# LSimon95/megatts2

Measured on AMD Instinct MI355X. Metric: mel-frames/sec (whole node), higher is better.
Workload: dtype f32; 1 GPU; C3: B=32/GPU x 1 GPU, Np=70, Tp=431, Tm=431; stages vqpe+mrte+adm+plm+decoder+vocoder; forced durations; weights=synthetic (name-seeded), parallelism=dp1 (utterance shards, one RCCL all-gather of mels per step)

## Files before the change

include/megatts2_hip.h:

```cpp
#ifndef MEGATTS2_HIP_H
#define MEGATTS2_HIP_H

#include <stddef.h>
#include <stdint.h>

#ifdef __cplusplus
extern "C" {
#endif

typedef struct mt2_model mt2_model;

typedef struct mt2_config {
    int32_t mel_bins, mrte_hidden, mrte_kernel, mrte_stride, mrte_n_layer, mrte_n_stack, mrte_n_block;
    int32_t content_ff_dim, content_n_heads, content_n_layers, phone_vocab;
    int32_t vq_mel_bins, vq_stride, vq_hidden, vq_kernel, vq_n_layers, vq_n_stacks, vq_n_blocks, vq_bins, vq_dim;
    int32_t dec_kernel, dec_hidden, dec_n_stack, dec_n_block;
    int32_t plm_layers, plm_heads, plm_vq_dim, plm_tc_dim, plm_bins;
    int32_t adm_layers, adm_heads, adm_emb_dim, adm_tc_dim, adm_tc_emb_dim;
    int32_t hg_in_dim, hg_init_channels, hg_n_up, hg_up_rates[8], hg_up_kernels[8];
    int32_t hg_n_res, hg_res_kernels[4], hg_res_dilations[4][3];
    float hg_slope;
    int32_t max_positions;
    int32_t hg_inference_padding;
    int32_t hg_reflect_pad;
// ... 158 lines not shown

#define MT2_LIMITER_FIELDS 24
#define MT2_LIMITER_TILE 1024
#define MT2_LIMITER_MAX_HALF_WINDOW 1024
#define MT2_LIMITER_MAX_PASSES 4
int mt2_limiter_query(int sample_rate, long long L, double window_ms, int* half_window, int* tile, long long* workspace_bytes);
int mt2_limiter_window(int sample_rate, double window_ms, float* w );
int mt2_limit_true_peak(mt2_model* m, void* stream, const float* wav , const int32_t* lens , int L_max, int B,
                        int sample_rate, double pre_gain_db, double ceiling_dbtp, double window_ms, float* out ,
                        float* gain , float* need , double* stats );
int mt2_loudness_normalize_limited(mt2_model* m, void* stream, const float* wav , const int32_t* lens , int L_max,
                                   int B, int sample_rate, double target_lufs, double ceiling_dbtp, double window_ms, int passes,
                                   float* out , float* gain , float* need ,
                                   double* stats );

#define MT2_RUN_PLM 1
#define MT2_RUN_VOCODER 2
#define MT2_SKIP_ADM 4
#define MT2_PROMPT_VQPE 8
int mt2_synthesize_batch(mt2_model* m, void* stream, const int64_t* phone, const int32_t* phone_lens ,
                         int Np_max, const float* prompt_mel, const int32_t* prompt_lens , int Tp_max,
                         int B, const int32_t* forced_dur , const int64_t* forced_codes, int Tq_cap,
                         int flags, float* mel, int Tm_cap, int32_t* mel_lens , int32_t* dur_out,
                         int64_t* codes_out, float* wav, int64_t* prompt_codes);

int mt2_synthesize_prompt_conditioned(mt2_model* m, void* stream, const int64_t* phone, const int32_t* phone_lens ,
                                      int Np_max, const float* prompt_mel, const int32_t* prompt_lens , int Tp_max, int B,
                                      const int64_t* prompt_phone, const int32_t* prompt_phone_lens , int Npp_max,
                                      const int32_t* prompt_dur , const int32_t* forced_dur , int Tq_cap, int flags,
                                      float* mel, int Tm_cap, int32_t* mel_lens , int32_t* dur_out, int64_t* codes_out,
                                      float* wav, int64_t* prompt_codes);
int mt2_synthesize_batch_sampled(mt2_model* m, void* stream, const int64_t* phone, const int32_t* phone_lens ,
                                 int Np_max, const float* prompt_mel, const int32_t* prompt_lens , int Tp_max,
                                 int B, const int32_t* forced_dur , const int64_t* forced_codes, int Tq_cap,
                                 int flags, float* mel, int Tm_cap, int32_t* mel_lens , int32_t* dur_out,
                                 int64_t* codes_out, float* wav, int64_t* prompt_codes, const mt2_sampling* sampling);
int mt2_synthesize_prompt_conditioned_sampled(mt2_model* m, void* stream, const int64_t* phone,
                                              const int32_t* phone_lens , int Np_max, const float* prompt_mel,
                                              const int32_t* prompt_lens , int Tp_max, int B,
                                              const int64_t* prompt_phone, const int32_t* prompt_phone_lens ,
                                              int Npp_max, const int32_t* prompt_dur ,
                                              const int32_t* forced_dur , int Tq_cap, int flags, float* mel,
                                              int Tm_cap, int32_t* mel_lens , int32_t* dur_out, int64_t* codes_out,
                                              float* wav, int64_t* prompt_codes, const mt2_sampling* sampling);

int mt2_set_option(mt2_model* m, const char* name, int value);
int mt2_get_option(mt2_model* m, const char* name, int* value);
int mt2_set_ar_groups(mt2_model* m, int groups);

int mt2_set_profiling(mt2_model* m, int enable);
int mt2_last_stage_ms(mt2_model* m, const char** names, float* ms, int cap);

int mt2_op_gemm(void* stream, const float* X, int ldx, int Rx, const int32_t* rowbase, int a_mul, int shift0,
                int taps, int dil, int Cin, const float* W, int ldw, const float* bias, const float* R, int ldr,
                const int32_t* valid, float* C, int ldc, int M, int N, int pro_act, float pro_slope, int epi_act,
                float out_scale, int force_cfg);
int mt2_op_gemm_x6(void* stream, const float* X, int ldx, int Rx, int shift0, int taps, int dil, int Cin, const float* W,
                   const void* W3, const float* bias, const float* R, int ldr, const int32_t* valid, float* C, int ldc,
                   int M, int N, int pro_act, float pro_slope, int epi_act, int force_cfg);
int mt2_op_gemm_x3h(void* stream, const float* X, int ldx, int Rx, int shift0, int taps, int dil, int Cin, const float* W,
                    const void* W3, const void* Wh, const float* wh_inv, const float* bias, const float* R, int ldr,
                    const int32_t* valid, float* C, int ldc, int M, int N, int pro_act, float pro_slope, int epi_act, int force_cfg,
                    int32_t* range_flag);
int mt2_x3h_split(const float* W, long long rows, long long row_len, uint16_t* planes, float* inv);
int mt2_x3h_group_planes(long long row_len, long long w_off, long long ldw, long long strideW, long long groups, int32_t* form,
                         long long* wh_off, long long* wh_ldb, long long* wh_gstride, long long* inv_off, long long* wh_inv_stride);
typedef struct mt2_gemm_desc {
    int32_t struct_bytes;
    const float* X; long long strideX; int32_t ldx, Rx;
    const int32_t* rowbase; int32_t a_mul, shift0, taps, dil, Cin;
    const float* W; long long strideW; int32_t ldw;
    const void* W3; long long w3_plane;
    const void* Wh; const float* wh_inv; long long wh_ldb, wh_gstride, wh_inv_stride;
    int32_t a_planes;
    const float* bias; long long strideB;
    const float* R; long long strideR; int32_t ldr;
    const int32_t* valid;
    float* C; long long strideC; int32_t ldc;
    int32_t M, N, groups;
    int32_t pro_act; float pro_slope; int32_t epi_act; float out_scale;
    int32_t force_cfg;
    int32_t* range_flag;
    int32_t* cfg_out;
} mt2_gemm_desc;
int mt2_op_gemm_grouped(void* stream, const mt2_gemm_desc* d);
int mt2_x3h_guard(mt2_model* m, int* tripped);
int mt2_op_gemm_x6_ln(void* stream, const float* X, int ldx, int Rx, int a_mul, int shift0, const float* W, const void* W3,
                      const float* bias, const float* R, int ldr, float* C, int ldc, int M, int N, int K, int epi_act,
                      int force_cfg, float* stat_out, int32_t* stat_nt, int32_t* stat_w, const float* ln_stat, int ln_nt,
                      int ln_w, const float* ln_s, float ln_eps);
int mt2_op_tile_major(void* stream, const float* W, int N, int K, float* out);
int mt2_op_gemm_tm(void* stream, const float* X, long long x_gstride, int ldx, int Rx, int a_mul, int shift0, const float* Wtm,
                   int Kw, int n0, int k0, long long w_gstride, int groups, const float* bias, const float* R, int ldr,
                   const int32_t* valid, float* C, long long c_gstride, int ldc, int M, int N, int K, int pro_act, float pro_slope,
                   int epi_act, const float* ln_gamma, const float* ln_beta, float ln_eps);
int mt2_op_gemm_tm_pairs(void* stream, const float* X, int ldx, int Rx, int a_mul, int shift0, const float* Wtm, int Kw,
                         const float* bias, const float* R, int ldr, float* C, int ldc, int M, int N, int K, int epi_act,
                         const float* ln_gamma, const float* ln_beta, float ln_eps, float* stat_out, const float* ln_stat, int ln_nt);
int mt2_op_layernorm(void* stream, const float* x, int ldx, const float* gamma, const float* beta, const float* R1,
                     int ldr1, const int32_t* valid, float* out, int ldo, int M, int C, float eps, int act);
int mt2_op_layernorm_ex(void* stream, const float* x, int ldx, const float* gamma, const float* beta, int rows_per_group,
                        const float* R1, int ldr1, int r1_rows, const float* R2, int ldr2, const int32_t* valid, int valid_rows,
                        float* out, int ldo, int M, int C, float eps, int act, int out_planes, int32_t* x3h_flag);
int mt2_op_ln_reduce(void* stream, const float* parts, long long pstride, int S, const float* bias, const float* R, int ldr,
                     const float* gamma, const float* beta, float* xout, int ldx, float* hout, int ldh, int M, int C, float eps,
                     int h_planes, int32_t* x3h_flag);
int mt2_op_row(void* stream, const char* op, void* const* ptrs, int nptrs, const long long* ints, int nints, const float* flts,
               int nflts);
int mt2_op_sample_rows(void* stream, const float* logits, int ld, int N, int A, const mt2_sampling* s, const uint64_t* seeds_dev,
                       const int32_t* positions_dev, int64_t* out);
int mt2_op_sample_mix_rows(void* stream, const float* logits, int ld, int N, int A, const mt2_sampling* s,
                           const uint64_t* seeds_dev, const int32_t* positions_dev, const float* gamma_dev, int64_t* out);
int mt2_op_attention(void* stream, const float* Q, int ldq, const float* K, int ldk, const float* V, int ldv,
                     float* O, int ldo, const int32_t* q_start, const int32_t* q_len, const int32_t* kv_start,
                     const int32_t* kv_len, int B, int H, int D, int max_qlen, float scale);
int mt2_op_attention_tuned(void* stream, const float* Q, int ldq, const float* K, int ldk, const float* V, int ldv,
                           float* O, int ldo, const int32_t* q_start, const int32_t* q_len, const int32_t* kv_start,
                           const int32_t* kv_len, int B, int H, int D, int max_qlen, float scale, int lds_min_qlen,
                           int lds_waves, int x6_min_qlen, int max_kvlen);
int mt2_op_attention_x3h(void* stream, const float* Q, int ldq, const float* K, int ldk, const float* V, int ldv,
                         float* O, int ldo, const int32_t* q_start, const int32_t* q_len, const int32_t* kv_start,
                         const int32_t* kv_len, int B, int H, int D, int max_qlen, float scale, int lds_waves, int max_kvlen,
                         int32_t* range_flag);
enum { MT2_ATTN_NONE = 0, MT2_ATTN_GENERIC = 1, MT2_ATTN_REG = 2, MT2_ATTN_DS = 3, MT2_ATTN_LDS = 4, MT2_ATTN_X6 = 5, MT2_ATTN_X3H = 6 };
typedef struct mt2_attn_desc {
    int32_t struct_bytes;
    const float* Q; int32_t ldq;
    const float* K; int32_t ldk;
    const float* V; int32_t ldv;
    float* O; int32_t ldo;
    const int32_t* q_start; const int32_t* q_len; const int32_t* kv_start; const int32_t* kv_len; const int32_t* o_start;
    int32_t u_qstride, u_qlen, u_kvstride, u_kvlen, u_ostride;
    int32_t B, H, D, max_qlen, max_kvlen; float scale;
    int32_t lds_min_qlen, x6_min_qlen, lds_waves, ds_short, x3h, o_planes;
    int32_t* range_flag;
    int32_t* kernel_out;
} mt2_attn_desc;
int mt2_op_attention_desc(void* stream, const mt2_attn_desc* d);
int mt2_attention_route(const mt2_attn_desc* d, int32_t* err, int32_t* kernel, int32_t* tmpl, int32_t* launch, long long* lds);
int mt2_gemm_trace_begin(mt2_model* m);
int mt2_gemm_trace_end(mt2_model* m, int cap, const char** names, int64_t* launches, double* flops, double* ms);
int mt2_gemm_trace_shapes(mt2_model* m, char* buf, int cap, int top);
int mt2_form_log_begin(mt2_model* m);
int mt2_form_log_end(mt2_model* m, char* buf, int cap);
int mt2_gemm_config_count(void);
const char* mt2_gemm_config_name(int idx);
int mt2_gemm_route(int M, int N, int K, int taps, int dil, int groups, int pro_act, int operands, int misaligned, int force_cfg,
                   int x3h, int* err, int* cfg, int* variant, long long* lds, int* planes);
int mt2_conv_pair_route(int R, int C, int taps, int dil, int flags, int pair_fuse, int x3h, int* err, long long* lds, int* grid,
                        int* block, int* bm, int* bmo);
int mt2_op_conv_pair(void* stream, const float* X, int ldx, int R, int C, int taps, int dil, float slope, const void* Wh1,
                     const float* inv1, const float* bias1, const void* Wh2, const float* inv2, const float* bias2,
                     const int32_t* valid, float* Y, int ldy, int pair_fuse, int32_t* range_flag);
int mt2_up_mrf_route(int R, int ch, int stride, int flags, int up_fuse, int x3h, int off, int* err, long long* lds, int* grid, int* block,
                     int* bm);
int mt2_op_up_mrf(void* stream, const float* X0, const float* X1, const float* X2, int ldx, int R, int ch, float scale, float slope,
                  const void* Wh, const float* inv, const float* bias, const int32_t* valid, float* Y, int ldy, int up_fuse,
                  int32_t* range_flag);
int mt2_op_gemm_x3h_ln(void* stream, const float* X, int ldx, int Rx, int a_mul, int shift0, const float* W, const void* W3,
                       const void* Wh, const float* wh_inv, const float* bias, const float* R, int ldr, float* C, int ldc, int M, int N,
                       int K, int epi_act, int force_cfg, float* stat_out, int32_t* stat_nt, int32_t* stat_w, const float* ln_stat,
                       int ln_nt, int ln_w, const float* ln_s, float ln_eps);
int mt2_bench_gemm(void* stream, int M, int N, int K, int taps, int dil, int flags, int force_cfg, int iters,
                   int w_copies, float* avg_ms, char* cfg_name, int cfg_name_cap, double* sustained_ghz);

#ifdef __cplusplus
}
#endif
#endif
```

megatts2_amd/csrc/capi.inc:

```

#include <climits>

namespace mt2 {
extern thread_local std::string g_last_error;
void finalize_model(mt2_model& m);
}

using namespace mt2;

#define MT2_API_BEGIN try {
#define MT2_API_END                                 \
    ::CallScope::verdict_of_open_call();            \
    return 0;                                       \
    }                                               \
    catch (const std::exception& e) {               \
        g_last_error = e.what();                    \
        return -1;                                  \
    }                                               \
    catch (...) {                                   \
        g_last_error = "unknown error";             \
        return -1;                                  \
    }

enum Need { NEED_G = 1, NEED_ADM = 2, NEED_PLM = 4, NEED_VOC = 8 };
// ... 232 lines not shown
    need((m.hg_post.k - 1) / 2);
    return (int)gap;
}

int mt2_workspace_query(const mt2_model* m, int B, int Np_max, int Tp_max, int Tm_cap, int flags, size_t* bytes) {
    MT2_API_BEGIN
    MT2_REQUIRE(m != nullptr && bytes != nullptr && B >= 1 && Np_max >= 1 && Tp_max >= 1 && Tm_cap >= 1, "bad arguments");
    const mt2_config& cfg = m->cfg;
    auto rows = [&](long long len, int gap) { return (long long)gap + (long long)B * (len + gap); };
    auto enc = [&](long long M, long long d, long long ff) {
        return M * (5 * d + ff + 128) + std::max(256ll * 32 * 64 + 16ll * 32 * d, 8 * M * d) + 7 * 64;
    };
    auto ar = [&](long long d, long long ff, long long L, int stage_groups) {
        const long long M = (long long)B * L;
        const int G = std::max(1, std::min(stage_groups > 0 ? stage_groups : m->ar_groups, B));
        return M * d + 3 * M * d + (long long)B * d + G * enc(0, d, ff) + enc(M + 2ll * B * G, d, ff) - enc(0, d, ff);
    };
    const long long H = cfg.mrte_hidden, st = cfg.mrte_stride;
    const long long FR = rows(Tp_max, prompt_mel_gap(cfg)), XR = rows((Tp_max - 1) / st + 1, mel_context_gap(cfg)), PR = rows(Np_max, phone_gap(cfg));
    long long f = 0;
    f += 16 * (FR + XR + PR) + 64;
    f += FR * cfg.mel_bins + FR * H + 4 * FR * H * cfg.mrte_n_layer + XR * H * cfg.mrte_n_layer;
    f += 4 * XR * H * cfg.mrte_n_layer + 2 * XR * H;
    f += PR * H + enc(PR, H, cfg.content_ff_dim) + 2 * XR * H + 2 * PR * H;
    if (!(flags & MT2_SKIP_ADM)) {
        f += PR * cfg.adm_tc_emb_dim + (long long)B * (Np_max + 1) + 8ll * B;
        f += ar(cfg.adm_emb_dim + cfg.adm_tc_emb_dim, 4ll * cfg.adm_emb_dim, Np_max, m->adm_groups);
    }
    const long long DR = rows(Tm_cap, decoder_gap(cfg)), DIN = H + cfg.vq_dim, Tq = (Tm_cap + cfg.vq_stride - 1) / cfg.vq_stride;
    f += 8 * DR + 4ll * B * Tq + DR * DIN + (long long)B * Tq * H + (long long)B * Np_max;
    if (flags & MT2_RUN_PLM) {
        const long long d = cfg.plm_vq_dim + cfg.plm_tc_dim;
        f += 2ll * B * (Tq + 1) + 2ll * B * Tq + 8ll * B + (long long)B * cfg.plm_bins + 2ll * B;
        f += ar(d, 4 * d, Tq, m->plm_groups);
    }
    f += DR * cfg.dec_hidden * 5 + DR * cfg.mel_bins;
    if (flags & MT2_PROMPT_VQPE) {
        const long long VR = rows(Tp_max, vqpe_gap(cfg)), QR = rows((Tp_max + cfg.vq_stride - 1) / cfg.vq_stride, vqpe_gap(cfg));
        const long long C = cfg.vq_hidden, G = cfg.vq_n_layers;
        f += 16 * (VR + QR) + VR * cfg.mel_bins + VR * C + 4 * VR * C * G + G * QR * C + 4 * QR * C * G + QR * C;
        f += QR * cfg.vq_dim + QR * cfg.vq_bins + 2 * QR;
    }
    if (flags & MT2_RUN_VOCODER) {
        const long long pad = cfg.hg_inference_padding;
        long long R = rows(Tm_cap + 2 * pad, vocoder_gap(*m)), ch = cfg.hg_init_channels;
        f += 4 * R + R * cfg.mel_bins + R * ch;
        for (int i = 0; i < cfg.hg_n_up; ++i) {
            R *= cfg.hg_up_rates[i];
            ch /= 2;
            f += R + 14 * R * ch;
        }
        f += R + 4ll * B + 64;
    }
    *bytes = (size_t)f * sizeof(float) + (size_t)400 * 256 + ((size_t)8 << 20);
    MT2_API_END
}

static int* option_slot(mt2_model* m, const std::string& n) {
    if (n == "ar_groups") return &m->ar_groups;
    if (n == "adm_groups") return &m->adm_groups;
    if (n == "plm_groups") return &m->plm_groups;
    if (n == "force_gemm_config") return &m->opts.force_cfg;
    if (n == "t_ks4") return &m->opts.t_ks4;
    if (n == "t_ks2") return &m->opts.t_ks2;
    if (n == "t32") return &m->opts.t32;
    if (n == "t32x32") return &m->opts.t32x32;
    if (n == "t_x6_256") return &m->opts.t_x6_256;
    if (n == "t_x6_128") return &m->opts.t_x6_128;
    if (n == "t_x3h_128") return &m->opts.t_x3h_128;
    if (n == "x3h") return &m->opts.x3h;
    if (n == "x6_ks") return &m->opts.x6_ks;
    if (n == "voc_streams") return &m->opts.voc_streams;
    if (n == "ldr_prio") return &m->opts.ldr_prio;
    if (n == "skinny_rows") return &m->opts.skinny_rows;
    if (n == "skinny_nw") return &m->opts.skinny_nw;
    if (n == "skinny_pairs") return &m->opts.skinny_pairs;
    if (n == "attn_lds_min") return &m->opts.attn_lds_min;
    if (n == "attn_x6_min") return &m->opts.attn_x6_min;
    if (n == "ln_pairs_adm") return &m->opts.ln_pairs_adm;
    if (n == "ln_pairs_maxm") return &m->opts.ln_pairs_maxm;
    if (n == "a_planes") return &m->opts.a_planes;
    if (n == "pair_fuse") return &m->opts.pair_fuse;
    if (n == "up_fuse") return &m->opts.up_fuse;
    return nullptr;
}
static bool* option_flag(mt2_model* m, const std::string& n) {
    if (n == "splitk") return &m->opts.splitk;
    if (n == "stage_markers") return &m->opts.markers;
    if (n == "win_conv") return &m->opts.win_conv;
    if (n == "x6_conv") return &m->opts.x6_conv;
    if (n == "x6_gemm") return &m->opts.x6_gemm;
    if (n == "skinny_tm") return &m->opts.skinny_tm;
    if (n == "ldr64") return &m->opts.ldr64;
    return nullptr;
}
int mt2_set_option(mt2_model* m, const char* name, int value) {
    MT2_API_BEGIN
    MT2_REQUIRE(m != nullptr && name != nullptr, "null argument");
    std::lock_guard<std::mutex> lk(m->call_mutex);
    const std::string n(name);
    if (n == "ar_groups") MT2_REQUIRE(value >= 1 && value <= 8, "ar_groups must be in 1..8");
    if (int* p = option_slot(m, n)) *p = value;
    else if (bool* q = option_flag(m, n)) *q = value != 0;
    else throw Error("unknown option " + n);
    MT2_API_END
}
int mt2_get_option(mt2_model* m, const char* name, int* value) {
    MT2_API_BEGIN
    MT2_REQUIRE(m != nullptr && name != nullptr && value != nullptr, "null argument");
    const std::string n(name);
    if (int* p = option_slot(m, n)) *value = *p;
    else if (bool* q = option_flag(m, n)) *value = *q ? 1 : 0;
    else throw Error("unknown option " + n);
    MT2_API_END
}
int mt2_set_ar_groups(mt2_model* m, int groups) { return mt2_set_option(m, "ar_groups", groups); }
int mt2_set_profiling(mt2_model* m, int enable) {
    MT2_API_BEGIN
    MT2_REQUIRE(m != nullptr, "null model handle");
    m->profiling = enable != 0;
    MT2_API_END
}
int mt2_last_stage_ms(mt2_model* m, const char** names, float* ms, int cap) {
    if (!m) return -1;
    const int n = (int)m->stage_ms.size();
    for (int i = 0; i < n && i < cap; ++i) {
        names[i] = m->stage_names[i].c_str();
        ms[i] = m->stage_ms[i];
    }
    return n;
}

int mt2_mrte_tc_latent(mt2_model* m, void* stream, const int64_t* phone, const int32_t* phone_lens, int Np_max,
                       const float* mel, const int32_t* mel_lens, int Tp_max, int B, float* out) {
    MT2_API_BEGIN
    require_ready(m, NEED_G);
    MT2_REQUIRE(B >= 1, "empty batch");
    MT2_CALL(m, stream);
    const int H = m->cfg.mrte_hidden;
    TcResult r = tc_latent_rows(c, phone, phone_lens, Np_max, mel, mel_lens, Tp_max, B);
    IntPlan ip;
    const int o_map = plan_rowmap(ip, r.P, Np_max);
    ip.upload(c.ws, c.m.pinned(), c.s);
    MT2_HIP(hipMemsetAsync(out, 0, sizeof(float) * (size_t)B * Np_max * H, c.s));
    MT2_HIP(launch_unpack_rows(r.rows, H, H, Np_max, 0, ip.dev(o_map), out, r.P.R, c.s));
    ids_verdict(c);
    MT2_API_END
}

int mt2_mrte_mel_context(mt2_model* m, void* stream, const float* mel, const int32_t* mel_lens, int Tp_max, int B,
                         float* out, int Tc_max) {
    MT2_API_BEGIN
    require_ready(m, NEED_G);
    MT2_REQUIRE(B >= 1, "empty batch");
    MT2_CALL(m, stream);
    const mt2_config& cfg = m->cfg;
    IntPlan ip;
    MelPlan mp = plan_mel(ip, cfg, mel_lens, B, Tp_max, Tc_max);
    MT2_REQUIRE(mp.X.maxlen <= Tc_max, "Tc_max too small");
    ip.upload(c.ws, c.m.pinned(), c.s);
    bind_rows(ip, mp.oF, mp.F);
    bind_rows(ip, mp.oX, mp.X);
    float* xmel = c.ws.get<float>((size_t)mp.F.R * cfg.mel_bins);
    MT2_HIP(launch_pack_rows(mel, cfg.mel_bins, Tp_max, 0, ip.dev(mp.o_rowmapF), xmel, cfg.mel_bins, mp.F.R, c.s));
    float* ctx = mel_context_rows(c, xmel, cfg.mel_bins, mp.F, mp.X, ip.dev(mp.o_rowbase));
    const int H = cfg.mrte_hidden;
// ... 826 lines not shown
    float* xdec = rows + (size_t)pp.D.R * DIN;
    MT2_HIP(launch_gather_rows(tc.rows, H, ip.dev(pp.o_tcmap), rows, DIN, H, pp.D.R, c.s));
    MT2_HIP(launch_gather_rows(tc.rows, H, ip.dev(fp.o_tcmap), xdec, DIN, H, fp.D.R, c.s));
    float* cond = c.ws.get<float>((size_t)qr * H);
    MT2_HIP(launch_pool_max(rows, DIN, ip.dev(o_first), ip.dev(o_cnt), cond, H, H, qr, c.s));
    st.mark("regulate");
    join_vqpe_side(c);
    int64_t* cdev = codes_buffer(c, codes_out, B, Tq_cap);
    ArPrefix pre;
    pre.P = P; pre.data = prompt_codes; pre.stride = (Tp_max + pool - 1) / pool;
    plm_run(c, cond, H, q0, total.data(), B, cdev, Tq_cap, nullptr, 0, pre, sampling);
    st.mark("plm");
    decode_and_vocode(c, st, xdec, fp, ip, cdev, flags, mel, Tm_cap, wav, B);
    st.finish();
    MT2_API_END
}
int mt2_synthesize_prompt_conditioned(mt2_model* m, void* stream, const int64_t* phone, const int32_t* phone_lens, int Np_max,
                                      const float* prompt_mel, const int32_t* prompt_lens, int Tp_max, int B,
                                      const int64_t* prompt_phone, const int32_t* prompt_phone_lens, int Npp_max,
                                      const int32_t* prompt_dur, const int32_t* forced_dur, int Tq_cap, int flags, float* mel,
                                      int Tm_cap, int32_t* mel_lens, int32_t* dur_out, int64_t* codes_out, float* wav,
                                      int64_t* prompt_codes) {
    return mt2_synthesize_prompt_conditioned_sampled(m, stream, phone, phone_lens, Np_max, prompt_mel, prompt_lens, Tp_max, B,
                                                     prompt_phone, prompt_phone_lens, Npp_max, prompt_dur, forced_dur, Tq_cap,
                                                     flags, mel, Tm_cap, mel_lens, dur_out, codes_out, wav, prompt_codes,
                                                     nullptr);
}


int mt2_gemm_trace_begin(mt2_model* m) {
    MT2_API_BEGIN
    MT2_REQUIRE(m != nullptr, "null model handle");
    std::lock_guard<std::mutex> lk(m->call_mutex);
    for (auto& r : m->opts.trace) { (void)hipEventDestroy(r.e0); (void)hipEventDestroy(r.e1); }
    m->opts.trace.clear();
    m->opts.trace_on = true;
    MT2_API_END
}
int mt2_gemm_trace_end(mt2_model* m, int cap, const char** names, int64_t* launches, double* flops, double* ms) {
    if (!m) return -1;
    std::lock_guard<std::mutex> lk(m->call_mutex);
    return gemm_trace_collect(m->opts, cap, names, launches, flops, ms);
}
int mt2_gemm_trace_shapes(mt2_model* m, char* buf, int cap, int top) {
    if (!m || !buf || cap <= 0) return -1;
    std::lock_guard<std::mutex> lk(m->call_mutex);
    return gemm_trace_shapes(m->opts, buf, cap, top);
}
int mt2_form_log_begin(mt2_model* m) {
    MT2_API_BEGIN
    MT2_REQUIRE(m != nullptr, "null model handle");
    std::lock_guard<std::mutex> lk(m->call_mutex);
    m->form_log.clear();
    m->form_kind = nullptr;
    m->form_log_on = true;
    MT2_API_END
}
int mt2_form_log_end(mt2_model* m, char* buf, int cap) {
    if (!m || !buf || cap <= 0) return -1;
    std::lock_guard<std::mutex> lk(m->call_mutex);
    m->form_log_on = false;
    m->form_kind = nullptr;
    size_t need = 0;
    for (const std::string& l : m->form_log) need += l.size() + 1;
    int off = -1;
    if (need < (size_t)cap) {
        off = 0;
        for (const std::string& l : m->form_log) {
            std::memcpy(buf + off, l.data(), l.size());
            off += (int)l.size();
            buf[off++] = '\n';
        }
        buf[off] = 0;
    }
    m->form_log.clear();
    m->form_log.shrink_to_fit();
    return off;
}
int mt2_gemm_config_count(void) { return gemm_num_configs(); }
const char* mt2_gemm_config_name(int idx) { return gemm_config_name(idx); }

int mt2_gemm_route(int M, int N, int K, int taps, int dil, int groups, int pro_act, int operands, int misaligned, int force_cfg,
                   int x3h, int* err, int* cfg, int* variant, long long* lds, int* planes) {
    alignas(128) static char dummy[12 * 128];
    const auto ptr = [&](int slot, int bit) { return (void*)(dummy + 128 * slot + ((misaligned & bit) ? 4 : 0)); };
    GemmP p{};
    const int Cin = taps > 0 ? K / taps : K;
    p.X = (const float*)ptr(0, 512); p.ldx = Cin; p.Rx = M + taps * dil; p.a_mul = 1; p.taps = taps; p.dil = dil; p.Cin = Cin;
    p.W = (const float*)ptr(1, 0); p.ldw = K; p.C = (float*)ptr(2, 1024); p.ldc = N; p.M = M; p.N = N; p.K = K; p.groups = groups;
    p.strideX = (long long)p.Rx * Cin; p.strideW = (long long)N * K; p.strideC = (long long)M * N; p.strideB = N; p.strideR = (long long)M * N;
    p.pro_act = pro_act; p.out_scale = 1.0f;
    if (operands & 1) p.W3 = ptr(3, 1);
    if (operands & 2) { p.Wh = ptr(4, 2); p.wh_inv = (const float*)ptr(5, 0); }
    if (operands & 4) { p.Wtm = (const float*)ptr(6, 4); p.tm_kb = K / 64; }
    if (operands & 8) p.stat_out = (float*)ptr(7, 8);
    if (operands & 16) { p.ln_stat = (const float*)ptr(8, 16); p.ln_g = p.ln_b = (const float*)ptr(9, 0); p.ln_w = 64; p.ln_nt = K / 64; }
    if (operands & 32) { p.R = (const float*)ptr(10, 32); p.ldr = N; }
    if (operands & 64) p.rowbase = (const int*)ptr(11, 64);
    p.a_planes = (operands & 128) ? 1 : 0;
    p.c_planes = (operands & 256) ? 1 : 0;
    EngineOpts o;
    o.force_cfg = force_cfg;
    o.x3h = x3h;
    const GemmRoute r = gemm_route(p, o);
    if (err) *err = (int)r.err;
    if (cfg) *cfg = r.cfg;
    if (variant) *variant = r.variant;
    if (lds) *lds = (long long)r.lds;
    if (planes) *planes = (gemm_takes_planes(p, o) ? 1 : 0) | (gemm_writes_planes(p, o) ? 2 : 0);
    return 0;
}

int mt2_conv_pair_route(int R, int C, int taps, int dil, int flags, int pair_fuse, int x3h, int* err, long long* lds, int* grid,
                        int* block, int* bm, int* bmo) {
    alignas(128) static char dummy[8 * 128];
    PairP p{};
    p.X = (const float*)dummy; p.ldx = C; p.R = R; p.C = C; p.taps = taps; p.dil = dil; p.slope = 0.1f;
    if (!(flags & 2)) { p.Wh1 = dummy + 128; p.inv1 = (const float*)(dummy + 256); p.Wh2 = dummy + 384; p.inv2 = (const float*)(dummy + 512); }
    p.bias1 = (const float*)(dummy + 640); p.bias2 = (const float*)(dummy + 768);
    p.wh_ldb = 4ll * (((long long)taps * C + 31) / 32 * 32);
    p.Y = (float*)(dummy + 896 + ((flags & 8) ? 4 : 0)); p.ldy = C;
    p.reflect = (flags & 1) ? 1 : 0;
    if ((flags & 4) && R > 0) p.ldx = (int)((((1ll << 31) / 4 + R - 1) / R + 3) & ~3ll);
    EngineOpts o;
    o.pair_fuse = pair_fuse;
    o.x3h = x3h;
    const PairRoute r = conv_pair_route(p, o);
    if (err) *err = (int)r.err;
    if (lds) *lds = (long long)r.lds;
    if (grid) *grid = (int)r.grid;
    if (block) *block = (int)r.block;
    if (bm) *bm = r.bm;
    if (bmo) *bmo = r.bmo;
    return 0;
}
int mt2_op_conv_pair(void* stream, const float* X, int ldx, int R, int C, int taps, int dil, float slope, const void* Wh1,
                     const float* inv1, const float* bias1, const void* Wh2, const float* inv2, const float* bias2,
                     const int32_t* valid, float* Y, int ldy, int pair_fuse, int32_t* range_flag) {
    MT2_API_BEGIN
    PairP p{};
    p.X = X; p.ldx = ldx; p.R = R; p.C = C; p.taps = taps; p.dil = dil; p.slope = slope;
    p.Wh1 = Wh1; p.inv1 = inv1; p.bias1 = bias1; p.Wh2 = Wh2; p.inv2 = inv2; p.bias2 = bias2;
    p.wh_ldb = 4ll * (((long long)taps * C + 31) / 32 * 32);
    p.valid = valid; p.Y = Y; p.ldy = ldy;
    EngineOpts o;
    o.pair_fuse = pair_fuse;
    o.x3h_flag = range_flag;
    MT2_HIP(launch_conv_pair(p, (hipStream_t)stream, &o));
    MT2_API_END
}

int mt2_up_mrf_route(int R, int ch, int stride, int flags, int up_fuse, int x3h, int off, int* err, long long* lds, int* grid, int* block,
                     int* bm) {
    alignas(128) static char dummy[8 * 128];
    UpMrfP p{};
    p.X0 = (const float*)dummy; p.X1 = (flags & 32) ? nullptr : (const float*)(dummy + 128); p.X2 = (const float*)(dummy + 256);
    p.ldx = ch; p.R = R; p.ch = ch; p.stride = stride; p.scale = 1.0f / 3.0f; p.slope = 0.1f;
    if (!(flags & 1)) { p.Wh = dummy + 384 + ((flags & 8) ? 16 : 0); p.inv = (const float*)(dummy + 512); }
    p.bias = (const float*)(dummy + 640 + ((flags & 128) ? 4 : 0));
    p.wh_ldb = 8ll * ch;
    p.Y = (float*)(dummy + 768 + ((flags & 4) ? 4 : 0)); p.ldy = ch;
    if ((flags & 2) && R > 0) p.ldx = (int)((((1ll << 31) / 4 + R - 1) / R + 3) & ~3ll);
    if (flags & 16) p.ldx = ch + 2;
    if (flags & 64) p.ldy = ch - 4;
    EngineOpts o;
    o.up_fuse = up_fuse;
    o.x3h = x3h;
    if (off & 1) o.win_conv = false;
    if (off & 2) o.x6_conv = false;
    if (off & 4) o.force_cfg = 0;
    if (off & 8) o.ldr64 = true;
    const UpMrfRoute r = up_mrf_route(p, o);
    if (err) *err = (int)r.err;
    if (lds) *lds = (long long)r.lds;
    if (grid) *grid = (int)r.grid;
    if (block) *block = (int)r.block;
    if (bm) *bm = r.bm;
    return 0;
}
int mt2_op_up_mrf(void* stream, const float* X0, const float* X1, const float* X2, int ldx, int R, int ch, float scale, float slope,
                  const void* Wh, const float* inv, const float* bias, const int32_t* valid, float* Y, int ldy, int up_fuse,
                  int32_t* range_flag) {
    MT2_API_BEGIN
    UpMrfP p{};
    p.X0 = X0; p.X1 = X1; p.X2 = X2; p.ldx = ldx; p.R = R; p.ch = ch; p.stride = 2; p.scale = scale; p.slope = slope;
    p.Wh = Wh; p.inv = inv; p.bias = bias; p.wh_ldb = 8ll * ch;
    p.valid = valid; p.Y = Y; p.ldy = ldy;
    EngineOpts o;
    o.up_fuse = up_fuse;
    o.x3h_flag = range_flag;
    MT2_HIP(launch_up_mrf(p, (hipStream_t)stream, &o));
    MT2_API_END
}

int mt2_op_gemm(void* stream, const float* X, int ldx, int Rx, const int32_t* rowbase, int a_mul, int shift0,
                int taps, int dil, int Cin, const float* W, int ldw, const float* bias, const float* R, int ldr,
                const int32_t* valid, float* C, int ldc, int M, int N, int pro_act, float pro_slope, int epi_act,
                float out_scale, int force_cfg) {
    MT2_API_BEGIN
    GemmP p{};
    p.X = X; p.ldx = ldx; p.Rx = Rx; p.rowbase = rowbase; p.a_mul = a_mul ? a_mul : 1; p.shift0 = shift0;
    p.taps = taps; p.dil = dil; p.Cin = Cin; p.W = W; p.ldw = ldw; p.bias = bias; p.R = R; p.ldr = ldr;
    p.valid = valid; p.C = C; p.ldc = ldc; p.M = M; p.N = N; p.K = taps * Cin; p.groups = 1;
    p.pro_act = pro_act; p.pro_slope = pro_slope; p.epi_act = epi_act; p.out_scale = out_scale;
    EngineOpts o;
    o.force_cfg = force_cfg;
    MT2_HIP(launch_gemm(p, (hipStream_t)stream, &o));
    MT2_API_END
}

int mt2_op_gemm_x6(void* stream, const float* X, int ldx, int Rx, int shift0, int taps, int dil, int Cin, const float* W,
                   const void* W3, const float* bias, const float* R, int ldr, const int32_t* valid, float* C, int ldc,
                   int M, int N, int pro_act, float pro_slope, int epi_act, int force_cfg) {
    MT2_API_BEGIN
    GemmP p{};
    p.X = X; p.ldx = ldx; p.Rx = Rx; p.a_mul = 1; p.shift0 = shift0; p.taps = taps; p.dil = dil; p.Cin = Cin; p.W = W;
    p.W3 = W3; p.ldw = taps * Cin; p.bias = bias; p.R = R; p.ldr = ldr; p.valid = valid; p.C = C; p.ldc = ldc; p.M = M;
    p.N = N; p.K = taps * Cin; p.groups = 1; p.pro_act = pro_act; p.pro_slope = pro_slope; p.epi_act = epi_act;
    p.out_scale = 1.0f;
    EngineOpts o;
    o.force_cfg = force_cfg;
    MT2_HIP(launch_gemm(p, (hipStream_t)stream, &o));
    MT2_API_END
}

int mt2_op_gemm_x3h(void* stream, const float* X, int ldx, int Rx, int shift0, int taps, int dil, int Cin, const float* W,
                    const void* W3, const void* Wh, const float* wh_inv, const float* bias, const float* R, int ldr,
                    const int32_t* valid, float* C, int ldc, int M, int N, int pro_act, float pro_slope, int epi_act, int force_cfg,
                    int32_t* range_flag) {
    MT2_API_BEGIN
    GemmP p{};
    p.X = X; p.ldx = ldx; p.Rx = Rx; p.a_mul = 1; p.shift0 = shift0; p.taps = taps; p.dil = dil; p.Cin = Cin; p.W = W;
    p.W3 = W3; p.Wh = Wh; p.wh_inv = wh_inv; p.ldw = taps * Cin; p.bias = bias; p.R = R; p.ldr = ldr; p.valid = valid; p.C = C;
    p.ldc = ldc; p.M = M; p.N = N; p.K = taps * Cin; p.groups = 1; p.pro_act = pro_act; p.pro_slope = pro_slope; p.epi_act = epi_act;
    p.out_scale = 1.0f;
    EngineOpts o;
    if (force_cfg >= 4000) { p.c_planes = 1; force_cfg -= 4000; }
    if (force_cfg >= 2000) { p.a_planes = 1; force_cfg -= 2000; }
    o.ldr64 = force_cfg >= 1000;
    o.force_cfg = force_cfg >= 1000 ? force_cfg - 1000 : force_cfg;
    o.x3h_flag = range_flag;
    MT2_HIP(launch_gemm(p, (hipStream_t)stream, &o));
    MT2_API_END
}
int mt2_x3h_split(const float* W, long long rows, long long row_len, uint16_t* planes, float* inv) {
    MT2_API_BEGIN
    MT2_REQUIRE(W && planes && inv && rows > 0 && row_len > 0, "bad arguments");
    x3h_split_rows(W, (size_t)rows, (size_t)row_len, planes, inv);
    MT2_API_END
}
int mt2_x3h_group_planes(long long row_len, long long w_off, long long ldw, long long strideW, long long groups, int32_t* form,
                         long long* wh_off, long long* wh_ldb, long long* wh_gstride, long long* inv_off, long long* wh_inv_stride) {
    MT2_API_BEGIN
    MT2_REQUIRE(row_len > 0 && w_off >= 0 && groups >= 1 && form && wh_off && wh_ldb && wh_gstride && inv_off && wh_inv_stride,
                "bad arguments");
    const X3hGroupPlanes g = x3h_group_planes(row_len, w_off, ldw, strideW, groups);
    *form = g.form; *wh_off = g.wh_off; *wh_ldb = g.wh_ldb; *wh_gstride = g.wh_gstride; *inv_off = g.inv_off;
    *wh_inv_stride = g.wh_inv_stride;
    MT2_API_END
}

int mt2_op_gemm_grouped(void* stream, const mt2_gemm_desc* d) {
    MT2_API_BEGIN
    MT2_REQUIRE(d != nullptr, "null descriptor");
    MT2_REQUIRE(d->struct_bytes == (int32_t)sizeof(mt2_gemm_desc), "descriptor size mismatch");
    if (d->cfg_out) *d->cfg_out = -1;
    GemmP p{};
    p.X = d->X; p.strideX = d->strideX; p.ldx = d->ldx; p.Rx = d->Rx;
    p.rowbase = d->rowbase; p.a_mul = d->a_mul; p.shift0 = d->shift0; p.taps = d->taps; p.dil = d->dil; p.Cin = d->Cin;
    p.W = d->W; p.strideW = d->strideW; p.ldw = d->ldw;
    p.W3 = d->W3; p.w3_plane = d->w3_plane;
    p.Wh = d->Wh; p.wh_inv = d->wh_inv; p.wh_ldb = d->wh_ldb; p.wh_gstride = d->wh_gstride; p.wh_inv_stride = d->wh_inv_stride;
    p.a_planes = d->a_planes;
    p.bias = d->bias; p.strideB = d->strideB; p.R = d->R; p.strideR = d->strideR; p.ldr = d->ldr; p.valid = d->valid;
    p.C = d->C; p.strideC = d->strideC; p.ldc = d->ldc;
    p.M = d->M; p.N = d->N; p.K = d->taps * d->Cin; p.groups = d->groups;
    p.pro_act = d->pro_act; p.pro_slope = d->pro_slope; p.epi_act = d->epi_act; p.out_scale = d->out_scale;
    MT2_REQUIRE(p.X && p.W && p.C && p.taps >= 1 && p.dil >= 1 && p.a_mul >= 1 && p.groups >= 1, "bad arguments");
    EngineOpts o;
    o.force_cfg = d->force_cfg;
    o.x3h_flag = d->range_flag;
    if (d->cfg_out) *d->cfg_out = gemm_route(p, o).cfg;
    MT2_HIP(launch_gemm(p, (hipStream_t)stream, &o));
    MT2_API_END
}

static int op_gemm_ln_impl(void* stream, const float* X, int ldx, int Rx, int a_mul, int shift0, const float* W, const void* W3,
                           const void* Wh, const float* wh_inv, const float* bias, const float* R, int ldr, float* C, int ldc, int M,
                           int N, int K, int epi_act, int force_cfg, float* stat_out, int32_t* stat_nt, int32_t* stat_w,
                           const float* ln_stat, int ln_nt, int ln_w, const float* ln_s, float ln_eps);
int mt2_op_gemm_x6_ln(void* stream, const float* X, int ldx, int Rx, int a_mul, int shift0, const float* W, const void* W3,
                      const float* bias, const float* R, int ldr, float* C, int ldc, int M, int N, int K, int epi_act,
                      int force_cfg, float* stat_out, int32_t* stat_nt, int32_t* stat_w, const float* ln_stat, int ln_nt,
                      int ln_w, const float* ln_s, float ln_eps) {
    return op_gemm_ln_impl(stream, X, ldx, Rx, a_mul, shift0, W, W3, nullptr, nullptr, bias, R, ldr, C, ldc, M, N, K, epi_act, force_cfg,
                           stat_out, stat_nt, stat_w, ln_stat, ln_nt, ln_w, ln_s, ln_eps);
}
int mt2_op_gemm_x3h_ln(void* stream, const float* X, int ldx, int Rx, int a_mul, int shift0, const float* W, const void* W3,
                       const void* Wh, const float* wh_inv, const float* bias, const float* R, int ldr, float* C, int ldc, int M, int N,
                       int K, int epi_act, int force_cfg, float* stat_out, int32_t* stat_nt, int32_t* stat_w, const float* ln_stat,
                       int ln_nt, int ln_w, const float* ln_s, float ln_eps) {
    return op_gemm_ln_impl(stream, X, ldx, Rx, a_mul, shift0, W, W3, Wh, wh_inv, bias, R, ldr, C, ldc, M, N, K, epi_act, force_cfg,
                           stat_out, stat_nt, stat_w, ln_stat, ln_nt, ln_w, ln_s, ln_eps);
}
static int op_gemm_ln_impl(void* stream, const float* X, int ldx, int Rx, int a_mul, int shift0, const float* W, const void* W3,
                           const void* Wh, const float* wh_inv, const float* bias, const float* R, int ldr, float* C, int ldc, int M,
                           int N, int K, int epi_act, int force_cfg, float* stat_out, int32_t* stat_nt, int32_t* stat_w,
                           const float* ln_stat, int ln_nt, int ln_w, const float* ln_s, float ln_eps) {
    MT2_API_BEGIN
    GemmP p{};
    p.Wh = Wh; p.wh_inv = wh_inv;
    p.X = X; p.ldx = ldx; p.Rx = Rx; p.a_mul = a_mul ? a_mul : 1; p.shift0 = shift0; p.taps = 1; p.dil = 1; p.Cin = K; p.W = W;
    p.W3 = W3; p.ldw = K; p.bias = bias; p.R = R; p.ldr = ldr; p.C = C; p.ldc = ldc; p.M = M; p.N = N; p.K = K; p.groups = 1;
    p.epi_act = epi_act; p.out_scale = 1.0f; p.stat_out = stat_out;
    if (ln_stat) { p.pro_act = 5; p.ln_stat = ln_stat; p.ln_nt = ln_nt; p.ln_w = ln_w; p.ln_g = ln_s; p.ln_eps = ln_eps; }
    EngineOpts o;
    o.ldr64 = force_cfg >= 1000;
    o.force_cfg = force_cfg >= 1000 ? force_cfg - 1000 : force_cfg;
    const hipError_t e = launch_gemm(p, (hipStream_t)stream, &o);
    MT2_REQUIRE(e != hipErrorNotSupported, "this tile configuration has no pair-fed LayerNorm form");
    MT2_HIP(e);
    if (stat_nt) *stat_nt = o.last_stat_nt;
    if (stat_w) *stat_w = o.last_stat_w;
    MT2_API_END
}

int mt2_op_tile_major(void* stream, const float* W, int N, int K, float* out) {
    MT2_API_BEGIN
    MT2_REQUIRE(W && out && N > 0 && K > 0 && N % 16 == 0 && K % 64 == 0, "tile-major layout needs N % 16 == 0 and K % 64 == 0");
    MT2_HIP(launch_tile_major(W, N, K, out, (hipStream_t)stream));
    MT2_API_END
}

int mt2_op_gemm_tm(void* stream, const float* X, long long x_gstride, int ldx, int Rx, int a_mul, int shift0, const float* Wtm,
                   int Kw, int n0, int k0, long long w_gstride, int groups, const float* bias, const float* R, int ldr,
                   const int32_t* valid, float* C, long long c_gstride, int ldc, int M, int N, int K, int pro_act, float pro_slope,
                   int epi_act, const float* ln_gamma, const float* ln_beta, float ln_eps) {
    MT2_API_BEGIN
    MT2_REQUIRE(X && Wtm && C && Kw % 64 == 0 && n0 % 16 == 0 && k0 % 64 == 0 && groups >= 1, "bad arguments");
    GemmP p{};
    p.X = X; p.strideX = x_gstride; p.ldx = ldx; p.Rx = Rx; p.a_mul = a_mul ? a_mul : 1; p.shift0 = shift0; p.taps = 1; p.dil = 1;
    p.Cin = K; p.K = K; p.W = nullptr; p.strideW = w_gstride; p.ldw = Kw; p.Wtm = Wtm; p.tm_n0 = n0 / 16; p.tm_k0 = k0 / 64;
    p.tm_kb = Kw / 64; p.bias = bias; p.R = R; p.ldr = ldr; p.valid = valid; p.C = C; p.strideC = c_gstride; p.ldc = ldc;
    p.M = M; p.N = N; p.groups = groups; p.pro_act = ln_gamma ? 3 : (pro_act & 0xff); p.pro_slope = pro_slope; p.epi_act = epi_act;
    p.sk_nw = (pro_act & 0x100) ? 8 : 16;
    p.out_scale = 1.0f; p.ln_g = ln_gamma; p.ln_b = ln_beta; p.ln_eps = ln_eps;
    MT2_REQUIRE(gemm_skinny_tm_eligible(p, 64), "shape not served by the tile-major weight-streaming kernel");
    MT2_HIP(launch_gemm_skinny_tm(p, (hipStream_t)stream));
    MT2_API_END
}

int mt2_op_gemm_tm_pairs(void* stream, const float* X, int ldx, int Rx, int a_mul, int shift0, const float* Wtm, int Kw,
                         const float* bias, const float* R, int ldr, float* C, int ldc, int M, int N, int K, int epi_act,
                         const float* ln_gamma, const float* ln_beta, float ln_eps, float* stat_out, const float* ln_stat, int ln_nt) {
    MT2_API_BEGIN
    MT2_REQUIRE(X && Wtm && C && Kw % 64 == 0, "bad arguments");
    GemmP p{};
    p.X = X; p.ldx = ldx; p.Rx = Rx; p.a_mul = a_mul ? a_mul : 1; p.shift0 = shift0; p.taps = 1; p.dil = 1; p.Cin = K; p.K = K;
    p.ldw = Kw; p.Wtm = Wtm; p.tm_kb = Kw / 64; p.bias = bias; p.R = R; p.ldr = ldr; p.C = C; p.ldc = ldc; p.M = M; p.N = N; p.groups = 1;
    p.pro_act = ln_gamma ? 3 : 0; p.epi_act = epi_act; p.out_scale = 1.0f; p.ln_g = ln_gamma; p.ln_b = ln_beta; p.ln_eps = ln_eps;
    p.stat_out = stat_out; p.ln_stat = ln_stat; p.ln_nt = ln_nt; p.ln_w = ln_stat ? 16 : 0;
    EngineOpts o;
    hipError_t e = launch_gemm(p, (hipStream_t)stream, &o);
    MT2_HIP(e);
    MT2_REQUIRE(!stat_out || o.last_stat_w == 16, "the launch did not take the tile-major route with the statistics epilogue");
    MT2_API_END
}

int mt2_op_layernorm(void* stream, const float* x, int ldx, const float* gamma, const float* beta, const float* R1,
                     int ldr1, const int32_t* valid, float* out, int ldo, int M, int C, float eps, int act) {
    MT2_API_BEGIN
    LnP p{};
    p.x = x; p.ldx = ldx; p.gamma = gamma; p.beta = beta; p.R1 = R1; p.ldr1 = ldr1; p.valid = valid;
    p.out = out; p.ldo = ldo; p.M = M; p.C = C; p.eps = eps; p.act = act >= 100 ? act - 100 : act;
    p.out_planes = act >= 100 ? 1 : 0;
    MT2_HIP(launch_layernorm(p, (hipStream_t)stream));
    MT2_API_END
}

int mt2_op_layernorm_ex(void* stream, const float* x, int ldx, const float* gamma, const float* beta, int rows_per_group,
                        const float* R1, int ldr1, int r1_rows, const float* R2, int ldr2, const int32_t* valid, int valid_rows,
                        float* out, int ldo, int M, int C, float eps, int act, int out_planes, int32_t* x3h_flag) {
    MT2_API_BEGIN
    LnP p{};
    p.x = x; p.ldx = ldx; p.gamma = gamma; p.beta = beta; p.rows_per_group = rows_per_group;
    p.R1 = R1; p.ldr1 = ldr1; p.r1_rows = r1_rows; p.R2 = R2; p.ldr2 = ldr2; p.valid = valid; p.valid_rows = valid_rows;
    p.out = out; p.ldo = ldo; p.M = M; p.C = C; p.eps = eps; p.act = act; p.out_planes = out_planes; p.x3h_flag = x3h_flag;
    MT2_HIP(launch_layernorm(p, (hipStream_t)stream));
    MT2_API_END
}

int mt2_op_ln_reduce(void* stream, const float* parts, long long pstride, int S, const float* bias, const float* R, int ldr,
                     const float* gamma, const float* beta, float* xout, int ldx, float* hout, int ldh, int M, int C, float eps,
                     int h_planes, int32_t* x3h_flag) {
    MT2_API_BEGIN
    LnReduceP p{};
    p.parts = parts; p.pstride = pstride; p.S = S; p.bias = bias; p.R = R; p.ldr = ldr; p.gamma = gamma; p.beta = beta;
    p.xout = xout; p.ldx = ldx; p.hout = hout; p.ldh = ldh; p.M = M; p.C = C; p.eps = eps; p.h_planes = h_planes;
    p.x3h_flag = x3h_flag;
// ... 192 lines not shown
int mt2_bench_gemm(void* stream, int M, int N, int K, int taps, int dil, int flags, int force_cfg, int iters,
                   int w_copies, float* avg_ms, char* cfg_name, int cfg_name_cap, double* sustained_ghz) {
    MT2_API_BEGIN
    MT2_REQUIRE(taps >= 1 && K % taps == 0 && (K / taps) % 4 == 0 && iters >= 1 && dil >= 1, "bad GEMM shape");
    if (w_copies < 1) w_copies = 1;
    hipStream_t s = (hipStream_t)stream;
    const int Cin = K / taps;
    float *X, *W, *C, *R = nullptr, *bias = nullptr;
    int* valid = nullptr;
    MT2_HIP(hipMalloc((void**)&X, sizeof(float) * ((size_t)M + taps * dil) * Cin));
    MT2_HIP(hipMalloc((void**)&W, sizeof(float) * (size_t)N * K * w_copies));
    MT2_HIP(hipMalloc((void**)&C, sizeof(float) * (size_t)M * N));
    std::vector<float> h(std::max(std::max(((size_t)M + taps * dil) * Cin, (size_t)N * K), (size_t)M * N));
    unsigned rng = 12345u;
    for (auto& v : h) { rng = rng * 1664525u + 1013904223u; v = ((rng >> 8) & 0xffff) / 32768.0f - 1.0f; }
    MT2_HIP(hipMemcpy(X, h.data(), sizeof(float) * ((size_t)M + taps * dil) * Cin, hipMemcpyHostToDevice));
    if (flags & 2) {
        MT2_HIP(hipMalloc((void**)&R, sizeof(float) * (size_t)M * N));
        MT2_HIP(hipMalloc((void**)&bias, sizeof(float) * (size_t)N));
        MT2_HIP(hipMalloc((void**)&valid, sizeof(int) * (size_t)M));
        MT2_HIP(hipMemcpy(R, h.data(), sizeof(float) * (size_t)M * N, hipMemcpyHostToDevice));
        MT2_HIP(hipMemcpy(bias, h.data(), sizeof(float) * (size_t)N, hipMemcpyHostToDevice));
        std::vector<int> ones(M, 1);
        MT2_HIP(hipMemcpy(valid, ones.data(), sizeof(int) * (size_t)M, hipMemcpyHostToDevice));
    }
    for (int i = 0; i < w_copies; ++i)
        MT2_HIP(hipMemcpy(W + (size_t)i * N * K, h.data(), sizeof(float) * (size_t)N * K, hipMemcpyHostToDevice));
    uint16_t* W3 = nullptr;
    const size_t wn = (size_t)N * K, wall = wn * w_copies;
    {
        std::vector<uint16_t> pl(3 * wall);
        for (size_t i = 0; i < wn; ++i) {
            float r = h[i];
            for (int k = 0; k < 3; ++k) {
                uint32_t bits;
                std::memcpy(&bits, &r, 4);
                bits &= 0xffff0000u;
                float top;
                std::memcpy(&top, &bits, 4);
                for (int cidx = 0; cidx < w_copies; ++cidx) pl[k * wall + cidx * wn + i] = (uint16_t)(bits >> 16);
                r -= top;
            }
        }
        MT2_HIP(hipMalloc((void**)&W3, pl.size() * sizeof(uint16_t)));
        MT2_HIP(hipMemcpy(W3, pl.data(), pl.size() * sizeof(uint16_t), hipMemcpyHostToDevice));
    }
    uint16_t* Wh = nullptr;
    float* wh_inv = nullptr;
    const size_t whn = (size_t)N * 2 * x3h_padded_k((size_t)K);
    {
        std::vector<uint16_t> one(whn), pl(whn * w_copies);
        std::vector<float> inv((size_t)N);
        x3h_split_rows(h.data(), (size_t)N, (size_t)K, one.data(), inv.data());
        for (int cidx = 0; cidx < w_copies; ++cidx) std::memcpy(pl.data() + cidx * whn, one.data(), whn * sizeof(uint16_t));
        MT2_HIP(hipMalloc((void**)&Wh, pl.size() * sizeof(uint16_t)));
        MT2_HIP(hipMemcpy(Wh, pl.data(), pl.size() * sizeof(uint16_t), hipMemcpyHostToDevice));
        MT2_HIP(hipMalloc((void**)&wh_inv, inv.size() * sizeof(float)));
        MT2_HIP(hipMemcpy(wh_inv, inv.data(), inv.size() * sizeof(float), hipMemcpyHostToDevice));
    }
    float* Wtm = nullptr;
    const bool tm = M <= 64 && taps == 1 && N % 16 == 0 && K % 64 == 0;
    if (tm) {
        MT2_HIP(hipMalloc((void**)&Wtm, sizeof(float) * wall));
        for (int i = 0; i < w_copies; ++i) MT2_HIP(launch_tile_major(W + (size_t)i * wn, N, K, Wtm + (size_t)i * wn, s));
    }
    GemmP p{};
    p.X = X; p.ldx = Cin; p.Rx = M + taps * dil; p.a_mul = 1; p.shift0 = 0; p.taps = taps; p.dil = dil; p.Cin = Cin;
    p.Wh = Wh; p.wh_inv = wh_inv;
    p.W = W; p.W3 = W3; p.w3_plane = (long long)wall; p.ldw = K; p.C = C; p.ldc = N; p.M = M; p.N = N; p.K = K; p.groups = 1;
    p.out_scale = 1.0f;
    if (tm) { p.Wtm = Wtm; p.tm_kb = K / 64; }
    if (flags & 1) { p.pro_act = ACT_LRELU; p.pro_slope = 0.1f; }
    p.R = R; p.ldr = N; p.bias = bias; p.valid = valid;
    unsigned long long* dbg = nullptr;
    if (flags & 4) {
        MT2_HIP(hipMalloc((void**)&dbg, 16 * sizeof(unsigned long long)));
        MT2_HIP(hipMemset(dbg, 0, 16 * sizeof(unsigned long long)));
        p.dbg = dbg;
    }
    EngineOpts o;
    o.force_cfg = force_cfg;
    if (flags & 16) o.ldr_prio = 0;
    if (flags & 32) o.x3h = 0;
    hipError_t e = launch_gemm(p, s, &o);
    hipEvent_t e0, e1;
    MT2_HIP(hipEventCreate(&e0));
    MT2_HIP(hipEventCreate(&e1));
    MT2_HIP(hipEventRecord(e0, s));
    for (int i = 0; i < iters && e == hipSuccess; ++i) {
        p.W = W + (size_t)(i % w_copies) * N * K;
        p.W3 = W3 + (size_t)(i % w_copies) * N * K;
        p.Wh = Wh + (size_t)(i % w_copies) * whn;
        if (tm) p.Wtm = Wtm + (size_t)(i % w_copies) * N * K;
        e = launch_gemm(p, s, &o);
    }
    MT2_HIP(hipEventRecord(e1, s));
    MT2_HIP(hipEventSynchronize(e1));
    float ms = 0.f;
    MT2_HIP(hipEventElapsedTime(&ms, e0, e1));
    if (avg_ms) *avg_ms = ms / iters;
    if (sustained_ghz) *sustained_ghz = 0.0;
    if (cfg_name && cfg_name_cap > 0) {
        std::strncpy(cfg_name, o.last_cfg, cfg_name_cap - 1);
        cfg_name[cfg_name_cap - 1] = 0;
    }
    if (dbg) {
        unsigned long long hd[16] = {0};
        (void)hipMemcpy(hd, dbg, sizeof(hd), hipMemcpyDeviceToHost);
        const double nkd = hd[6] ? (double)hd[6] : 1.0;
        if (hd[0] + hd[1] + hd[5])
        std::fprintf(stderr, "x6 phase cycles per chunk (one wave, %llu chunks): dma_wait %.0f barrier %.0f refill_issue %.0f "
                             "first_fetch %.0f fetch2+split %.0f mfma_steps %.0f\n",
                     hd[6], hd[0] / nkd, hd[1] / nkd, hd[2] / nkd, hd[3] / nkd, hd[4] / nkd, hd[5] / nkd);
        if (hd[11] + hd[12] + hd[13])
            std::fprintf(stderr, "loader wave 0, cycles per chunk: vmcnt_wait %.0f barrier %.0f issue %.0f\n", hd[11] / nkd, hd[12] / nkd, hd[13] / nkd);
        int wall_khz = 0, sclk_khz = 0;
        (void)hipDeviceGetAttribute(&wall_khz, hipDeviceAttributeWallClockRate, 0);
        (void)hipDeviceGetAttribute(&sclk_khz, hipDeviceAttributeClockRate, 0);
        if (hd[7] && wall_khz > 0 && (flags & 8) == 0 && (hd[9] || hd[10]))
            std::fprintf(stderr, "one workgroup: entry -> K loop %.2f us, K loop %.2f us, epilogue %.2f us (launch average %.2f us)\n",
                         hd[9] / (wall_khz * 1e-3), hd[7] / (wall_khz * 1e-3), hd[10] / (wall_khz * 1e-3), ms / iters * 1e3);
        if (hd[7] && wall_khz > 0 && sustained_ghz) *sustained_ghz = (double)hd[8] / ((double)hd[7] / (wall_khz * 1e3)) / 1e9;
        if (hd[7] && wall_khz > 0 && (flags & 8) == 0)
            std::fprintf(stderr, "clock probe: %llu shader cycles in %llu ticks of the %d kHz wall clock -> %.3f GHz sustained in "
                                 "the K loop (device max %d kHz)\n", hd[8], hd[7], wall_khz,
                         (double)hd[8] / ((double)hd[7] / (wall_khz * 1e3)) / 1e9, sclk_khz);
        (void)hipFree(dbg);
    }
    (void)hipEventDestroy(e0);
    (void)hipEventDestroy(e1);
    (void)hipFree(X);
    (void)hipFree(W);
    (void)hipFree(W3);
    (void)hipFree(Wh);
    (void)hipFree(wh_inv);
    if (Wtm) (void)hipFree(Wtm);
    (void)hipFree(C);
    if (R) (void)hipFree(R);
    if (bias) (void)hipFree(bias);
    if (valid) (void)hipFree(valid);
    MT2_HIP(e);
    MT2_API_END
}

}
```

megatts2_amd/csrc/gemm_common.h:

```cpp
#pragma once
#include "gemm_tiles.h"
#include "planes_store.h"
#include <type_traits>
#include <utility>

namespace mt2 {

typedef float f32x16 __attribute__((ext_vector_type(16)));
typedef float f32x4 __attribute__((ext_vector_type(4)));

template <int ACT>
__device__ __forceinline__ float apply_act(float v, float slope) {
    if (ACT == ACT_RELU) return fmaxf(v, 0.0f);
    if (ACT == ACT_LRELU) return fmaxf(v, v * slope);
    if (ACT == ACT_TANH) return tanhf(v);
    return v;
}

__device__ __forceinline__ float act_rt(int act, float v, float slope) {
    switch (act) {
        case ACT_RELU: return fmaxf(v, 0.0f);
        case ACT_LRELU: return v >= 0.0f ? v : v * slope;
        case ACT_TANH: return tanhf(v);
        case ACT_LOGCLAMP: return logf(fmaxf(v, slope));
// ... 69 lines not shown
    rs = ok ? 1.0f / sqrtf(m2 / ((float)p.ln_nt * w) + p.ln_eps) : 0.0f;
}

template <int TM, int TN, int EPG = 16>
__device__ __forceinline__ void epilogue(const GemmP& p, f32x16 (&acc)[TM][TN], int g, int mw, int nw, int lane,
                                         int esel = 0) {
    const float* __restrict__ bias = p.bias ? p.bias + (long long)g * p.strideB : nullptr;
    const float* __restrict__ R = p.R ? p.R + (long long)g * p.strideR : nullptr;
    float* __restrict__ C = p.C + (long long)g * p.strideC;
    const int epi_act = p.epi_act;
    const float epi_par = p.pro_slope;
    const float out_scale = p.out_scale;
#pragma unroll
    for (int j = 0; j < TN; ++j) {
        const int n = nw + j * 32 + (lane & 31);
        const bool nok = n < p.N;
        const float bv = (bias && nok) ? bias[n] : 0.0f;
#pragma unroll
        for (int i = 0; i < TM; ++i) {
#pragma unroll
            for (int e = 0; e < 16; ++e) {
                if (EPG < 16 && e / EPG != esel) continue;
                const int m = mw + i * 32 + (e & 3) + 8 * (e >> 2) + 4 * (lane >> 5);
                if (nok && m < p.M) {
                    float v = acc[i][j][e] + bv;
                    v = act_rt(epi_act, v, epi_par) * out_scale;
                    if (R) v += R[(long long)m * p.ldr + n];
                    if (p.valid && p.valid[m] == 0) v = 0.0f;
                    C[(long long)m * p.ldc + n] = v;
                }
            }
        }
    }
}

static __device__ __attribute__((aligned(16))) float g_zero16[4] = {0.f, 0.f, 0.f, 0.f};
static __device__ int g_one_i[4] = {1, 1, 1, 1};
template <int NE> struct EpiPre { float r[NE]; int v[NE]; float b; };
template <int NE>
__device__ __forceinline__ void epi_prefetch(const GemmP& p, EpiPre<NE>& q, int g, int mw, int nw, int lane, int e0) {
    const int n = nw + (lane & 31);
    const bool nok = n < p.N;
    const float* __restrict__ bias = p.bias ? p.bias + (long long)g * p.strideB + (nok ? n : 0) : g_zero16;
    const float* __restrict__ R = p.R ? p.R + (long long)g * p.strideR + (nok ? n : 0) : g_zero16;
    const long long ldr = p.R ? p.ldr : 0;
    const int* __restrict__ vp = p.valid ? p.valid : g_one_i;
    const int vs = p.valid ? 1 : 0;
    q.b = *bias;
#pragma unroll
    for (int i = 0; i < NE; ++i) {
        const int e = e0 + i;
        int m = mw + (e & 3) + 8 * (e >> 2) + 4 * (lane >> 5);
        m = m < p.M ? m : 0;
        q.r[i] = R[m * ldr];
        q.v[i] = vp[m * vs];
    }
}
template <int NE, bool STAT = false>
__device__ __forceinline__ void epilogue_pre(const GemmP& p, const float (&acc)[NE], const EpiPre<NE>& q, int g, int mw,
                                             int nw, int lane, int e0) {
    float* __restrict__ C = p.C + (long long)g * p.strideC;
    const int epi_act = p.epi_act;
    const float epi_par = p.pro_slope;
    const float out_scale = p.out_scale;
    const bool hasR = p.R != nullptr;
    const int n = nw + (lane & 31);
    const bool nok = n < p.N;
    float sv[STAT ? NE : 1], qv[STAT ? NE : 1];
#pragma unroll
    for (int i = 0; i < NE; ++i) {
        const int e = e0 + i;
        const int m = mw + (e & 3) + 8 * (e >> 2) + 4 * (lane >> 5);
        float v = 0.0f;
        if (nok && m < p.M) {
            v = acc[i] + q.b;
            v = act_rt(epi_act, v, epi_par) * out_scale;
            if (hasR) v += q.r[i];
            if (q.v[i] == 0) v = 0.0f;
            C[(long long)m * p.ldc + n] = v;
        }
        if constexpr (STAT) { sv[i] = v; qv[i] = v * v; }
    }
    if constexpr (STAT) emit_row_pairs<NE>(p, sv, qv, mw, nw >> 5, 32.0f, lane, e0);
}

template <int TM, int TN> struct EpiPreT { float r[TM][TN][16]; int v[TM][16]; float b[TN]; };
template <int TM, int TN>
__device__ __forceinline__ void epi_prefetch_t(const GemmP& p, EpiPreT<TM, TN>& q, int g, int mw, int nw, int lane) {
    const float* __restrict__ bias0 = p.bias ? p.bias + (long long)g * p.strideB : g_zero16;
    const float* __restrict__ R0 = p.R ? p.R + (long long)g * p.strideR : g_zero16;
    const long long ldr = p.R ? p.ldr : 0;
    const int* __restrict__ vp = p.valid ? p.valid : g_one_i;
    const int vs = p.valid ? 1 : 0;
#pragma unroll
    for (int j = 0; j < TN; ++j) {
        const int n = nw + j * 32 + (lane & 31);
        const int nc = (n < p.N && (p.bias || p.R)) ? n : 0;
        q.b[j] = bias0[p.bias ? nc : 0];
#pragma unroll
        for (int i = 0; i < TM; ++i)
#pragma unroll
            for (int e = 0; e < 16; ++e) {
                int m = mw + i * 32 + (e & 3) + 8 * (e >> 2) + 4 * (lane >> 5);
                m = m < p.M ? m : 0;
                q.r[i][j][e] = R0[m * ldr + (p.R ? nc : 0)];
            }
    }
#pragma unroll
    for (int i = 0; i < TM; ++i)
#pragma unroll
        for (int e = 0; e < 16; ++e) {
            int m = mw + i * 32 + (e & 3) + 8 * (e >> 2) + 4 * (lane >> 5);
            m = m < p.M ? m : 0;
            q.v[i][e] = vp[m * vs];
        }
}
template <int TM, int TN, bool STAT = false>
__device__ __forceinline__ void epilogue_pre_t(const GemmP& p, f32x16 (&acc)[TM][TN], const EpiPreT<TM, TN>& q, int g,
                                               int mw, int nw, int lane) {
    static_assert(!STAT || TM == 1, "row statistics: one 32-row block per wave");
    float* __restrict__ C = p.C + (long long)g * p.strideC;
    const int epi_act = p.epi_act;
    const float epi_par = p.pro_slope;
    const float out_scale = p.out_scale;
    const bool hasR = p.R != nullptr;
    float sv[STAT ? 16 : 1], qv[STAT ? 16 : 1];
    if constexpr (STAT) {
#pragma unroll
        for (int e = 0; e < 16; ++e) { sv[e] = 0.0f; qv[e] = 0.0f; }
    }
#pragma unroll
    for (int j = 0; j < TN; ++j) {
        const int n = nw + j * 32 + (lane & 31);
        const bool nok = n < p.N;
#pragma unroll
        for (int i = 0; i < TM; ++i)
#pragma unroll
            for (int e = 0; e < 16; ++e) {
                const int m = mw + i * 32 + (e & 3) + 8 * (e >> 2) + 4 * (lane >> 5);
                float v = 0.0f;
                if (nok && m < p.M) {
                    v = acc[i][j][e] + q.b[j];
                    v = act_rt(epi_act, v, epi_par) * out_scale;
                    if (hasR) v += q.r[i][j][e];
                    if (q.v[i][e] == 0) v = 0.0f;
                    C[(long long)m * p.ldc + n] = v;
                }
                if constexpr (STAT) { sv[e] += v; qv[e] += v * v; }
            }
    }
    if constexpr (STAT) emit_row_pairs<16>(p, sv, qv, mw, nw / (32 * TN), 32.0f * TN, lane, 0);
}

__device__ __forceinline__ float dpp_quad(float v, const int ctrl) {
    return __builtin_bit_cast(float, ctrl == 0xB1 ? __builtin_amdgcn_mov_dpp(__builtin_bit_cast(int, v), 0xB1, 0xf, 0xf, true)
                                                  : __builtin_amdgcn_mov_dpp(__builtin_bit_cast(int, v), 0x4E, 0xf, 0xf, true));
}
__device__ __forceinline__ bool epilogue_t4_ok(const GemmP& p) {
    return ((p.N | p.ldc | (p.R ? p.ldr : 0)) & 3) == 0 && (((unsigned long long)p.C | (unsigned long long)p.R | (unsigned long long)p.bias) & 15) == 0 &&
           ((p.strideC | p.strideR | p.strideB) & 3) == 0;
}
template <int TM, int TN, bool STAT = false, bool PLN = false>
__device__ __forceinline__ void epilogue_t4(const GemmP& p, f32x16 (&acc)[TM][TN], int g, int mw, int nw, int lane) {
    static_assert(!STAT || TM == 1, "row statistics: one 32-row block per wave");
    float* __restrict__ C = p.C + (long long)g * p.strideC;
    const int epi_act = p.epi_act;
// ... 128 lines not shown
```

megatts2_amd/csrc/gemm_dispatch.hip:

```cpp
#include "gemm_tiles.h"

#include <algorithm>
#include <atomic>
#include <cstdio>
#include <cstdlib>
#include <utility>
#include <vector>

namespace mt2 {


static const TileCfg kSkinnyRows[] = {
    { CFG_SKINNY32, 32, 32, 512, 0, "skinny32_f32", {} },
    { CFG_SKINNY64, 64, 32, 512, 0, "skinny64_f32", {} },
    { CFG_SKINNYTM32, 32, 32, 512, 0, "skinnytm32_f32", {} },
    { CFG_SKINNYTM64, 64, 32, 512, 0, "skinnytm64_f32", {} },
};
static const struct { int index; const char* name; } kRetired[] = {
    {0, "retired:128x128_2x2"}, {1, "retired:64x128_2x2"}, {2, "retired:128x64_2x2"}, {4, "retired:32x128_1x4"},
    {5, "retired:32x64_1x2"}, {6, "retired:128x32_4x1"}, {7, "retired:64x32_2x1"},
    {8, "retired:dma128x128_2x2_s3"}, {9, "retired:dma128x128_2x2_s4"}, {10, "retired:dma64x128_2x2_s4"},
    {11, "retired:dma64x64_2x2_s4"}, {13, "retired:dma32x128_1x4_s4"}, {14, "retired:dma32x64_1x2_s4"},
    {19, "retired:dma64x64_2x2_k2_s4"}, {21, "retired:dma32x64_1x2_k4_s3"}, {24, "retired:dma128x64_4x2_s4"},
    {25, "retired:dma128x64_4x2_s2"}, {26, "retired:dma64x64_2x2_k1_s2"}, {27, "retired:dma128x64_4x2_k2_s2"},
// ... 128 lines not shown
    }
    for (auto& r : tr) { (void)hipEventDestroy(r.e0); (void)hipEventDestroy(r.e1); }
    tr.clear();
    return ok ? n : -1;
}

template <typename F>
static hipError_t traced_launch(EngineOpts* opts, int cfg, const GemmP& p, hipStream_t s, F&& launch) {
    if (opts) opts->last_cfg = gemm_config_name(cfg);
    if (!(opts && opts->trace_on)) return launch();
    TraceRec r;
    r.cfg = cfg;
    r.flops = 2.0 * p.M * p.N * p.K * p.groups;
    r.M = p.M; r.N = p.N; r.K = p.K; r.groups = p.groups;
    if (hipEventCreate(&r.e0) != hipSuccess || hipEventCreate(&r.e1) != hipSuccess) return hipErrorUnknown;
    (void)hipEventRecord(r.e0, s);
    const hipError_t e = launch();
    (void)hipEventRecord(r.e1, s);
    opts->trace.push_back(r);
    return e;
}


static bool win_eligible(const GemmP& p) {
    return p.taps >= 2 && !p.rowbase && p.a_mul == 1 && p.groups == 1 && p.N == p.Cin &&
           (p.Cin == 32 || p.Cin == 64 || p.Cin == 128) && (p.taps - 1) * p.dil <= 64 && p.pro_act < PRO_LN;
}
static int choose_cfg(const GemmP& p, const EngineOpts& o) {
    const bool forced = o.force_cfg >= 0 && o.force_cfg < kNumCfgs;
    const bool x3h_ok = p.Wh && p.wh_inv;
    if (o.win_conv && win_eligible(p) && !forced) {
        int bi = p.Cin == 32 ? CFG_WIN256x32 : (p.Cin == 64 ? CFG_WIN256x64 : CFG_WIN128x128);
        if (o.x6_conv && p.W3) {
            bi = paired(kX6Form, bi);
            if ((o.x3h & 4) && x3h_ok) bi = paired(kX3hForm, bi);
        }
        return bi;
    }
    if (forced) return o.force_cfg;
    const long long t32 = (long long)((p.M + 31) / 32) * ((p.N + 63) / 64) * p.groups;
    const long long t32x32 = (long long)((p.M + 31) / 32) * ((p.N + 31) / 32) * p.groups;
    const long long t64 = (long long)((p.M + 63) / 64) * ((p.N + 63) / 64) * p.groups;
    const long long t128 = (long long)((p.M + 127) / 128) * ((p.N + 127) / 128) * p.groups;
    const long long t256 = (long long)((p.M + 255) / 256) * ((p.N + 127) / 128) * p.groups;
    int bi = CFG_DMA64x64_S3;
    if (p.N <= 32) bi = CFG_DMA128x32_S4;
    else if (p.N <= 64 && t128 >= 400) bi = CFG_DMA256x64_S3;
    else if (p.N <= 256 && t128 >= 400) bi = CFG_DMA128x128_S4;
    else if (t256 >= 400 || (t256 >= 200 && t256 <= 256)) bi = CFG_DMA256x128_S3;
    else if (t128 >= 400 || (t128 >= 200 && t128 <= 256)) bi = CFG_DMA128x128_S4;
    else if (t32x32 <= o.t32x32 && p.K >= 512) bi = CFG_DMA32x32_K8;
    else if (t32 <= o.t32) bi = CFG_DMA32x64_K4;
    else if (t64 <= o.t_ks4) bi = CFG_DMA64x64_K4;
    else if (t64 <= o.t_ks2) bi = CFG_DMA64x64_K2;
    if (o.x6_gemm && p.W3 && (p.K & 7) == 0 && (p.ldw & 7) == 0 && (p.pro_act < PRO_LN || p.pro_act == PRO_LNX) && p.N > 64) {
        const bool h1 = (o.x3h & 1) && x3h_ok;
        if (t256 >= o.t_x6_256) bi = CFG_X6LDR256x128;
        else if (t128 >= (h1 ? o.t_x3h_128 : o.t_x6_128)) bi = CFG_X6LDR128x128;
        if (o.x6_ks && p.taps == 1) {
            if (bi == CFG_DMA32x64_K4 && p.K % (BK * 4) == 0 && o.x6_ks != 5) bi = paired(kX6Form, bi);
            else if ((bi == CFG_DMA64x64_K4 || bi == CFG_DMA64x64_K2) && p.K % (BK * 2) == 0) bi = paired(kX6Form, bi);
            else if ((o.x6_ks == 2 || o.x6_ks == 4) && bi == CFG_DMA32x32_K8 && p.K % (BK * 8) == 0) bi = paired(kX6Form, bi);
        }
    }
    if ((o.x3h & 1) && x3h_ok && (bi == CFG_X6LDR128x128 || bi == CFG_X6LDR256x128)) bi = paired(kX3hForm, bi);
    if ((o.x3h & 2) && x3h_ok && cfg_table().row[bi]->pipe == PIPE_X6 && cfg_table().row[bi]->x6_ks) bi = paired(kX3hForm, bi);
    return bi;
}


static bool a_planes_ok(const GemmP& p, const TileCfg& c, bool stat) {
    return c.pipe == PIPE_X3H && !c.win_qs && p.pro_act == ACT_NONE && !stat && (p.Cin % BK) == 0 && (p.ldx % BK) == 0 &&
           !(p.groups > 1 && (p.strideX % BK) != 0) && p.a_mul == 1 && !p.rowbase && !(((unsigned long long)p.X) & 127);
}
static bool c_planes_ok(const GemmP& p, const TileCfg& c, bool stat) {
    return c.pipe == PIPE_X3H && !c.x6_ks && !c.win_qs && p.groups == 1 && !p.R && !stat && (p.N & 31) == 0 && (p.ldc & 31) == 0 &&
           (((unsigned long long)p.C) & 127) == 0 && (((unsigned long long)p.bias) & 15) == 0 && ((p.strideC | p.strideB) & 3) == 0 && p.Wh && p.wh_inv && p.M > 64;
}
static long long wh_ldb_of(const GemmP& p) { return p.wh_ldb ? p.wh_ldb : 4ll * ((p.ldw + 31) / 32 * 32); }
static long long wh_gstride_of(const GemmP& p) { return p.groups > 1 && p.wh_gstride == 0 ? p.strideW * 4 : p.wh_gstride; }

GemmRoute gemm_route(const GemmP& p, const EngineOpts& o) {
    GemmRoute r{hipSuccess, -1, V_NONE, 0, 0, 0};
    const auto fail = [&r](hipError_t e) { r.err = e; r.lds = 0; r.stat_nt = r.stat_w = 0; return r; };
    if (p.M <= 0 || p.N <= 0 || p.groups <= 0) return r;
    if ((p.Cin & 3) || (p.ldx & 3) || (p.ldw & 3) || p.K != p.taps * p.Cin) return fail(hipErrorInvalidValue);
    if (p.pro_act < 0 || p.pro_act > PRO_LNX) return fail(hipErrorInvalidValue);
    if (p.c_planes && p.M <= 64) return fail(hipErrorNotSupported);
    if (p.pro_act == PRO_LNX && (p.taps != 1 || p.groups != 1 || !p.ln_g || !p.ln_stat || p.ln_nt < 2 || p.ln_nt > 32 ||
                                 (p.ln_nt & 1) || p.ln_w <= 0 || p.ln_nt * p.ln_w != p.K || (((unsigned long long)p.ln_stat) & 15)))
        return fail(hipErrorInvalidValue);
    const bool sk_forced = o.force_cfg == CFG_SKINNY32 || o.force_cfg == CFG_SKINNY64;
    const bool tm_forced = o.force_cfg == CFG_SKINNYTM32 || o.force_cfg == CFG_SKINNYTM64;
    if (tm_forced || (!p.a_planes && o.skinny_tm && o.skinny_rows > 0 && o.force_cfg < 0 &&
                      gemm_skinny_tm_eligible(p, o.skinny_rows))) {
        if (!gemm_skinny_tm_eligible(p, 64)) return fail(hipErrorInvalidValue);
        r.cfg = p.M <= 32 ? CFG_SKINNYTM32 : CFG_SKINNYTM64;
        if (p.stat_out) {
            const int nt = p.N / 16;
            if (p.groups == 1 && (nt & 1) == 0 && nt <= 64 && ((((unsigned long long)p.stat_out) & 15) == 0)) { r.stat_nt = nt; r.stat_w = 16; }
        }
        return r;
    }
    if (sk_forced || (o.skinny_rows > 0 && o.force_cfg < 0 && gemm_skinny_eligible(p, o.skinny_rows))) {
        if (!gemm_skinny_eligible(p, 64)) return fail(hipErrorInvalidValue);
        r.cfg = p.M <= 32 ? CFG_SKINNY32 : CFG_SKINNY64;
        return r;
    }
    r.cfg = choose_cfg(p, o);
    const TileCfg* c = cfg_table().row[r.cfg];
    if (!c) return fail(hipErrorNotSupported);
    const bool x3h = c->pipe == PIPE_X3H, x3h_ldr = x3h && !c->x6_ks && !c->win_qs;
    const bool has_lnx = c->stat_w && c->fn[V_LNX];
    if (p.pro_act == PRO_LNX && !has_lnx) return fail(hipErrorNotSupported);
    bool stat = p.stat_out != nullptr;
    if (x3h_ldr && (p.pro_act == PRO_LNX || stat)) {
        const bool t4 = ((p.N | p.ldc | (p.R ? p.ldr : 0)) & 3) == 0 && ((p.strideC | p.strideR | p.strideB) & 3) == 0 &&
                        (((unsigned long long)p.C | (unsigned long long)p.R | (unsigned long long)p.bias) & 15) == 0;
        if (!t4) {
            if (p.pro_act == PRO_LNX) return fail(hipErrorNotSupported);
            stat = false;
        }
    }
    if (stat) {
        const int nt = c->stat_w ? p.N / c->stat_w : 0;
        stat = has_lnx && (p.pro_act == ACT_NONE || p.pro_act == PRO_LNX) && p.groups == 1 && p.N % c->stat_w == 0 && nt >= 2 &&
               nt <= 32 && (nt & 1) == 0 && ((((unsigned long long)p.stat_out) & 15) == 0);
        if (stat) { r.stat_w = c->stat_w; r.stat_nt = nt; }
    }
    if (p.a_planes && !a_planes_ok(p, *c, stat)) return fail(hipErrorNotSupported);
    if (p.c_planes && !c_planes_ok(p, *c, stat)) return fail(hipErrorNotSupported);
    if (p.pro_act == PRO_LN || p.pro_act == PRO_LNA) return fail(hipErrorNotSupported);
    r.variant = p.a_planes ? V_APLANES : ((p.pro_act == PRO_LNX || stat) ? V_LNX : (GemmVariant)p.pro_act);
    r.lds = c->lds;
    if (r.variant == V_LNX && !c->x6_ks) r.lds += (size_t)c->bm * 2 * sizeof(float);
    if (x3h) {
        if (!p.Wh || !p.wh_inv || (p.K & 7) || (p.ldw & 7)) return fail(hipErrorInvalidValue);
        if ((((unsigned long long)p.Wh) & 127) || (wh_ldb_of(p) & 127) || (wh_gstride_of(p) & 127)) return fail(hipErrorInvalidValue);
    } else if (c->pipe == PIPE_X6 && (!p.W3 || (p.K & 7) || (p.ldw & 7))) return fail(hipErrorInvalidValue);
    if (c->x6_ks && (p.taps != 1 || p.K % (BK * c->x6_ks) != 0)) return fail(hipErrorInvalidValue);
    if (c->win_qs) {
        if (!win_eligible(p) || p.Cin != 32 * c->win_qs) return fail(hipErrorInvalidValue);
        const int wrp = (c->bm + (p.taps - 1) * p.dil + 7) & ~7;
        r.lds = c->lds + (size_t)c->win_qs * wrp * BK * sizeof(float);
    }
    if (!c->fn[r.variant]) return fail(hipErrorNotSupported);
    return r;
}

static GemmP normalise(GemmP p) {
    if (p.taps <= 0) p.taps = 1;
    if (p.groups <= 0) p.groups = 1;
    if (p.a_mul == 0) p.a_mul = 1;
    p.K = p.taps * p.Cin;
    if (p.ldw == 0) p.ldw = p.K;
    return p;
}
bool gemm_takes_planes(const GemmP& p_in, const EngineOpts& o) {
    const GemmP p = normalise(p_in);
    if (!(o.x3h & 3) || o.force_cfg >= 0 || p.M <= 64 || !p.Wh || !p.wh_inv) return false;
    const TileCfg* c = cfg_table().row[choose_cfg(p, o)];
    return a_planes_ok(p, *c, p.stat_out != nullptr) && c->fn[V_APLANES] != nullptr;
}
bool gemm_writes_planes(const GemmP& p_in, const EngineOpts& o) {
    const GemmP p = normalise(p_in);
    if (!(o.x3h & 1) || o.force_cfg >= 0 || p.M <= 64) return false;
    return c_planes_ok(p, *cfg_table().row[choose_cfg(p, o)], p.stat_out != nullptr);
}

static std::atomic<unsigned long long> g_attr_done[kNumCfgs][kGemmVariants];

hipError_t launch_gemm(const GemmP& p_in, hipStream_t s, EngineOpts* opts) {
    static const EngineOpts kDefaults;
    const EngineOpts& o = opts ? *opts : kDefaults;
    const GemmRoute r = gemm_route(p_in, o);
    if (r.cfg < 0 && r.err == hipSuccess) return hipSuccess;
    if (opts) { opts->last_stat_nt = r.stat_nt; opts->last_stat_w = r.stat_w; opts->last_sk_nw = 0; }
    if (r.err != hipSuccess) return r.err;
    GemmP p = p_in;
    if (!r.stat_nt) p.stat_out = nullptr;
    p.stat_nt = r.stat_nt; p.stat_w = r.stat_w;
    if (r.cfg == CFG_SKINNYTM32 || r.cfg == CFG_SKINNYTM64) {
        p.sk_nw = o.skinny_nw;
        if (opts) opts->last_sk_nw = gemm_skinny_tm_waves(p);
        return traced_launch(opts, r.cfg, p, s, [&] { return launch_gemm_skinny_tm(p, s); });
    }
    if (r.cfg == CFG_SKINNY32 || r.cfg == CFG_SKINNY64) return traced_launch(opts, r.cfg, p, s, [&] { return launch_gemm_skinny(p, s); });
    const TileCfg* c = cfg_table().row[r.cfg];
    if (c->pipe == PIPE_X3H) {
        p.wh_ldb = wh_ldb_of(p);
        p.wh_gstride = wh_gstride_of(p);
        p.x3h_flag = o.x3h_flag;
    }
    if (c->pipe == PIPE_X6 && p.w3_plane == 0) p.w3_plane = (long long)p.N * p.ldw;
    const GemmKernel fn = c->fn[r.variant];
    const size_t lds_attr = c->win_qs ? c->lds + (size_t)c->win_qs * ((c->bm + 64 + 7) & ~7) * BK * sizeof(float) : r.lds;
    const hipError_t e = dyn_lds_once(g_attr_done[r.cfg][r.variant], reinterpret_cast<const void*>(fn), lds_attr);
    if (e != hipSuccess) return e;
    const int tiles = ((p.M + c->bm - 1) / c->bm) * ((p.N + c->bn - 1) / c->bn);
    p.epi_t4 = 1;
    p.ldr_prio = o.ldr_prio;
    p.ldr64 = o.ldr64 ? 1 : 0;
    const dim3 grid(tiles, 1, p.groups), block(c->threads);
    return traced_launch(opts, r.cfg, p, s, [&] {
        hipLaunchKernelGGL(fn, grid, block, r.lds, s, p);
        return hipGetLastError();
    });
}

}
```

megatts2_amd/csrc/gemm_tiles.h:

```cpp
#pragma once
#include "mt2_kernels.h"

namespace mt2 {

constexpr int BK = 32;
constexpr int PRO_LN = 3;
constexpr int PRO_LNA = 4;
constexpr int PRO_LNX = 5;

enum GemmVariant : int {
    V_NONE, V_RELU, V_LRELU,
    V_APLANES,
    V_LNX,
    kGemmVariants
};
static_assert((int)V_NONE == ACT_NONE && (int)V_RELU == ACT_RELU && (int)V_LRELU == ACT_LRELU, "the activation variants are indexed by Act");

enum GemmPipe : int { PIPE_F32, PIPE_X6, PIPE_X3H };

enum CfgIndex : int {
    CFG_64x64 = 3,
    CFG_DMA64x64_S3 = 12, CFG_DMA128x32_S4 = 15, CFG_DMA256x128_S3 = 16, CFG_DMA128x128_S4 = 17,
    CFG_DMA64x64_K2 = 18, CFG_DMA64x64_K4 = 20, CFG_DMA32x64_K4 = 22, CFG_DMA256x64_S3 = 23, CFG_DMA32x32_K8 = 28,
    CFG_WIN256x32 = 30, CFG_WIN256x64 = 31, CFG_WIN128x128 = 32,
    CFG_X6WIN256x32 = 34,
    CFG_X6LDR256x128 = 51, CFG_X6LDR128x128 = 55,
    CFG_X6WINL256x64 = 58, CFG_X6WINL128x128 = 59,
    CFG_X6KS32x64_K4 = 84, CFG_X6KS64x64_K2 = 85, CFG_X6KS32x32_K8 = 86,
    CFG_SKINNY32 = 87, CFG_SKINNY64 = 88, CFG_SKINNYTM32 = 89, CFG_SKINNYTM64 = 90,
    CFG_X3HKS32x64_K4 = 95, CFG_X3HKS64x64_K2 = 96, CFG_X3HKS32x32_K8 = 97,
    CFG_X3HWIN256x32 = 98, CFG_X3HWIN256x64 = 99, CFG_X3HWIN128x128 = 100,
    CFG_X3HLDR128x128 = 103,
    kNumCfgs = 106
};

typedef void (*GemmKernel)(GemmP);
struct TileCfg {
    CfgIndex index;
    int bm, bn, threads;
    size_t lds;
    const char* name;
    GemmKernel fn[kGemmVariants];
    GemmPipe pipe = PIPE_F32;
    int win_qs = 0;
    int x6_ks = 0;
    int stat_w = 0;
};
struct TileRows { const TileCfg* rows; int n; };
TileRows gemm_f32_tile_rows();
TileRows gemm_x3h_tile_rows();

}
```

megatts2_amd/csrc/gemm_x3h.hip:

```cpp
#include "gemm_common.h"

#include <atomic>

#ifndef MT2_X3H_ABLATE
#define MT2_X3H_ABLATE 0
#endif
#define MT2_ABL_NOINGEST (MT2_X3H_ABLATE == 2 || MT2_X3H_ABLATE == 5 || MT2_X3H_ABLATE == 6 || MT2_X3H_ABLATE == 7)
#define MT2_ABL_NOSPLIT (MT2_X3H_ABLATE == 3 || MT2_X3H_ABLATE == 5 || MT2_X3H_ABLATE == 6)
#define MT2_ABL_NOBARRIER (MT2_X3H_ABLATE == 6 || MT2_X3H_ABLATE == 7)
#ifdef MT2_X3H_NO_BUFFER_LOADS
#define MT2_BUFFER_LOADS false
#else
#define MT2_BUFFER_LOADS true
#endif

namespace mt2 {

typedef _Float16 f16x8 __attribute__((ext_vector_type(8)));
typedef _Float16 f16x2 __attribute__((ext_vector_type(2)));
typedef float f32x2 __attribute__((ext_vector_type(2)));
typedef unsigned u32x4 __attribute__((ext_vector_type(4)));

constexpr float kX3hLoScale = 2048.0f, kX3hLoInv = 1.0f / 2048.0f, kX3hMaxIn = 65504.0f;

// ... 427 lines not shown
                }
                if (i == TM - 1) {
                    if constexpr (!last) {
                        if (b == 0 && !MT2_ABL_NOBARRIER) {
                            __builtin_amdgcn_s_barrier();
                            asm volatile("" ::: "memory");
                        }
                        fetch_a(b, sa);
                        __builtin_amdgcn_sched_barrier(0);
                        asm volatile("s_waitcnt lgkmcnt(%0)" :: "n"(N1) : "memory");
                    } else {
                        asm volatile("s_waitcnt lgkmcnt(0)" ::: "memory");
                    }
                    tie_a(b ^ 1);
                    if (TM == 1) tie_b(b);
                    __builtin_amdgcn_sched_barrier(0);
                }
                const bool more = s + 1 < FS || !last;
                if (more) {
                    const int s2 = (s + 1) % FS, b2 = s2 / TM, i2 = s2 % TM;
                    if (b2 == b) tie(b2, i2);
                    split2_f16<PRO>(ra[b2][i2][0], ra[b2][i2][1], pro_slope, pln[(s + 1) & 1][0], pln[(s + 1) & 1][1], amax);
                    products(b, i, pln[s & 1]);
                    pattern();
                    __builtin_amdgcn_sched_barrier(0);
                } else {
                    products(b, i, pln[s & 1]);
                    __builtin_amdgcn_sched_barrier(0);
                }
                if constexpr (!last) {
                    if (i == TM - 1) {
                        fetch_b(b, sb);
                        __builtin_amdgcn_sched_barrier(0);
                    }
                }
            }
            stn = stn + 1 == NST ? 0 : stn + 1;
        };
        for (int c = 0; c + 1 < nk; ++c) chunk(std::false_type{});
        chunk(std::true_type{});
    }
    }
    unsigned long long t_loop_end = 0;
    if (probe) {
        t_loop_end = __builtin_amdgcn_s_memrealtime();
        if (lane == 0) {
            p.dbg[6] = (unsigned long long)nk;
            p.dbg[7] = t_loop_end - treal0;
            p.dbg[8] = __builtin_readcyclecounter() - tcyc0;
        }
    }
    MT2_X3H_GUARD_RAISE(p, amax, lane);
#pragma unroll
    for (int i = 0; i < TM; ++i)
#pragma unroll
        for (int j = 0; j < TN; ++j)
#pragma unroll
            for (int e = 0; e < 16; ++e) acc[i][j][e] = __builtin_fmaf(acl[i][j][e], kX3hLoInv, acc[i][j][e]) * inv_s[j];

    if constexpr (LNXOK) {
        if (lnx) {
#pragma unroll
            for (int j = 0; j < TN; ++j) {
                const int n = n0 + wn * WTN + j * 32 + (lane & 31);
                const float s_n = n < p.N ? p.ln_g[n] : 0.0f;
#pragma unroll
                for (int e = 0; e < 16; ++e) {
                    const float2 st2 = reinterpret_cast<const float2*>(lnstat)[wm * WTM + (e & 3) + 8 * (e >> 2) + 4 * half];
                    acc[0][j][e] = st2.y * (acc[0][j][e] - st2.x * s_n);
                }
            }
        }
        if (p.stat_out) epilogue_t4<TM, TN, true>(p, acc, g, m0 + wm * WTM, n0 + wn * WTN, lane);
        else epilogue_t4<TM, TN, false, true>(p, acc, g, m0 + wm * WTM, n0 + wn * WTN, lane);
    } else if (p.epi_t4 && epilogue_t4_ok(p)) epilogue_t4<TM, TN, false, true>(p, acc, g, m0 + wm * WTM, n0 + wn * WTN, lane);
    else epilogue<TM, TN>(p, acc, g, m0 + wm * WTM, n0 + wn * WTN, lane);
    if (probe) {
        __builtin_amdgcn_s_waitcnt(0);
        const unsigned long long t_end = __builtin_amdgcn_s_memrealtime();
        if (lane == 0) p.dbg[10] = t_end - t_loop_end;
    }
}

template <int BM, int BN, int WGM, int WGN, int KS, int NL, int NST, int PRO>
__global__ __launch_bounds__((WGM * WGN * KS + NL) * 64) void gemm_x3h_ks_kernel(GemmP p) {
    constexpr int NW = WGM * WGN;
    constexpr int NWC = NW * KS;
    constexpr int PA = BM / 8, PB = BN / 8;
    constexpr int PG = PA + PB, PT = PG * KS;
    constexpr int LW = PT / NL;
    constexpr int STAGE_A = BM * BK * 4, STAGE_B = PB * 1024, STAGE = STAGE_A + STAGE_B;
    constexpr int EPG = 16 / KS;
    static_assert(BM == 32 * WGM && BN == 32 * WGN, "one 32x32 tile per wave");
    static_assert(PT % NL == 0 && 16 % KS == 0 && NST >= 2 && (NST - 2) * LW < 64 && NWC + NL <= 16, "config");
    static_assert(KS * NST * STAGE >= NWC * 16 * 64 * 4 || KS == 1, "the K-group reduction reuses the ring");

    extern __shared__ __attribute__((aligned(16))) float smem[];
    char* ring = reinterpret_cast<char*>(smem);
    const int tid = threadIdx.x, lane = tid & 63;
    const int wave_all = __builtin_amdgcn_readfirstlane(tid >> 6);
    const int g = blockIdx.z;
    const unsigned long long t_entry = p.dbg ? __builtin_amdgcn_s_memrealtime() : 0ull;
    const int ntm = (p.M + BM - 1) / BM, ntn = (p.N + BN - 1) / BN, nt = ntm * ntn;
    const int bid = blockIdx.x;
    const int xcd = bid & 7, q = nt >> 3, r = nt & 7;
    const int tile = (xcd < r ? xcd * (q + 1) : r * (q + 1) + (xcd - r) * q) + (bid >> 3);
    const bool nmajor = p.M < p.N;
    const int m0 = (nmajor ? tile % ntm : tile / ntn) * BM, n0 = (nmajor ? tile / ntm : tile % ntn) * BN;
    const int nr = p.K / (BK * KS);

    if (wave_all >= NWC) {
        loader_priority(p.ldr_prio);
        const int lw = wave_all - NWC;
        const char* __restrict__ Xb = reinterpret_cast<const char*>(p.X + (long long)g * p.strideX);
        const char* __restrict__ Wb = reinterpret_cast<const char*>(p.Wh) + (long long)g * p.wh_gstride;
        const char* zero = reinterpret_cast<const char*>(g_zero16);
        const char* base[LW];
        long long rowb[LW];
        int ldsoff[LW];
        int grp[LW];
#pragma unroll
        for (int j = 0; j < LW; ++j) {
            const int pi = j * NL + lw, kg = pi / PG, w = pi - kg * PG;
            grp[j] = kg;
            if (w < PA) {
                const int m = m0 + w * 8 + (lane >> 3);
                int src = kInvalidRow;
                if (m < p.M) src = p.rowbase ? p.rowbase[m] : m * p.a_mul + p.shift0;
                const int kl = ((lane & 7) ^ ((w * 4 + (lane >> 4)) & 7)) * 4;
                base[j] = Xb; ldsoff[j] = w * 1024;
                rowb[j] = (unsigned)src < (unsigned)p.Rx ? ((long long)src * p.ldx + kl) * 4 : -1;
            } else {
                const int bp = w - PA;
                const int nl = bp * 8 + (lane >> 3), n = n0 + nl;
                const int sl = (lane & 7) ^ ((nl >> 1) & 7);
                base[j] = Wb; ldsoff[j] = STAGE_A + bp * 1024;
                rowb[j] = n < p.N ? (long long)n * p.wh_ldb + sl * 16 : -1;
            }
        }
        wait_vmcnt<0>();
        constexpr unsigned kOut = 0x80000000u;
        const bool fast32 = MT2_BUFFER_LOADS && !p.ldr64 && (long long)p.Rx * p.ldx * 4 + (long long)p.K * 4 < 0x7fffffffll && (long long)p.N * p.wh_ldb < 0x7fffffffll;
        const __amdgpu_buffer_rsrc_t rs_x = __builtin_amdgcn_make_buffer_rsrc(const_cast<char*>(Xb), 0, (int)kOut, 0x00020000);
        const __amdgpu_buffer_rsrc_t rs_w = __builtin_amdgcn_make_buffer_rsrc(const_cast<char*>(Wb), 0, (int)kOut, 0x00020000);
        unsigned vo[LW];
#pragma unroll
        for (int j = 0; j < LW; ++j) vo[j] = rowb[j] >= 0 ? (unsigned)rowb[j] + (unsigned)grp[j] * (BK * 4) : kOut;
        auto issue = [&](int rd, int st) __attribute__((always_inline)) {
            if (fast32) {
                const int so = rd * KS * BK * 4;
#pragma unroll
                for (int j = 0; j < LW; ++j) {
                    const bool is_a = base[j] == Xb;
                    __builtin_amdgcn_raw_ptr_buffer_load_lds(is_a ? rs_x : rs_w,
                                                             (__attribute__((address_space(3))) void*)(ring + (grp[j] * NST + st) * STAGE + ldsoff[j]),
                                                             16, (int)vo[j], so, 0, 0);
                }
                return;
            }
#pragma unroll
            for (int j = 0; j < LW; ++j) {
                const long long kb = (long long)(rd * KS + grp[j]) * BK * 4;
                const char* src = rowb[j] >= 0 ? base[j] + rowb[j] + kb : zero;
                __builtin_amdgcn_global_load_lds((const __attribute__((address_space(1))) void*)src,
                                                 (__attribute__((address_space(3))) void*)(ring + (grp[j] * NST + st) * STAGE + ldsoff[j]),
                                                 16, 0, 0);
            }
        };
#pragma unroll
        for (int st = 0; st < NST - 1; ++st)
            if (st < nr) issue(st, st);
#ifdef MT2_PHASE_TIMING
        const bool lprobe = p.dbg != nullptr && bid == (int)(gridDim.x / 2) && lw == 0;
        unsigned long long lacc[3] = {0, 0, 0}, lprev = lprobe ? __builtin_readcyclecounter() : 0ull;
#define MT2_LT(i_) do { if (lprobe) { const unsigned long long t_ = __builtin_readcyclecounter(); lacc[i_] += t_ - lprev; lprev = t_; } } while (0)
#else
#define MT2_LT(i_) do { } while (0)
#endif
        int st = 0;
        for (int rd = 0; rd < nr; ++rd) {
            if (rd + NST - 2 < nr) wait_vmcnt<(NST - 2) * LW>();
            else wait_vmcnt<0>();
            MT2_LT(0);
            __builtin_amdgcn_s_barrier();
            MT2_LT(1);
            if (rd + NST - 1 < nr) issue(rd + NST - 1, st == 0 ? NST - 1 : st - 1);
            MT2_LT(2);
            st = st + 1 == NST ? 0 : st + 1;
        }
#ifdef MT2_PHASE_TIMING
        if (lprobe && lane == 0) { p.dbg[11] = lacc[0]; p.dbg[12] = lacc[1]; p.dbg[13] = lacc[2]; }
#endif
#undef MT2_LT
        return;
    }

    const int kg = wave_all / NW, wave = wave_all % NW;
    const int wm = wave / WGN, wn = wave % WGN;
    EpiPre<EPG> pre;
    epi_prefetch<EPG>(p, pre, g, m0 + wm * 32, n0 + wn * 32, lane, kg * EPG);
    float inv_s;
    {
        const int n = n0 + wn * 32 + (lane & 31);
        inv_s = (p.wh_inv + (long long)g * p.wh_inv_stride)[n < p.N ? n : 0];
    }
    float ln_mu = 0.0f, ln_rs = 0.0f;
    const bool lnx = PRO == PRO_LNX && p.pro_act == PRO_LNX;
    if (lnx) lnx_row_stats<2>(p, m0 + wm * 32 + (lane & 31), lane >> 5, 32, ln_mu, ln_rs);
    f32x16 acc, acl;
#pragma unroll
    for (int e = 0; e < 16; ++e) { acc[e] = 0.0f; acl[e] = 0.0f; }
    const float pro_slope = p.pro_slope;
    const int half = lane >> 5;
    const unsigned lds0 = (unsigned)(unsigned long long)(__attribute__((address_space(3))) char*)ring + (unsigned)(kg * NST) * STAGE;
    const int swza = (lane >> 1) & 7;
    const unsigned a_lane = lds0 + ((wm * 32 + (lane & 31)) * BK) * 4;
    const int nrow = wn * 32 + (lane & 31);
    const int swzb = (nrow >> 1) & 7;
    const unsigned b_lane = lds0 + STAGE_A + nrow * 128;
    unsigned koffa[2][2], koffb[2][2];
#pragma unroll
    for (int b = 0; b < 2; ++b) {
        koffa[b][0] = (unsigned)(((b * 4 + half * 2) ^ swza) * 16);
        koffa[b][1] = (unsigned)(((b * 4 + half * 2 + 1) ^ swza) * 16);
        koffb[b][0] = (unsigned)(((b * 2 + half) ^ swzb) * 16);
        koffb[b][1] = (unsigned)(((4 + b * 2 + half) ^ swzb) * 16);
    }
    float amax = 0.0f;
    f32x4 ra[2][2];
    u32x4 rb[2][2], pln[2];
    auto fetch = [&](int b, unsigned sa, unsigned sb) {
        ra[b][0] = lds_read_b128(sa + (PRO == PRO_APL ? (unsigned)(((b * 2 + half) ^ swza) * 16) : koffa[b][0]));
        ra[b][1] = lds_read_b128(sa + (PRO == PRO_APL ? (unsigned)(((4 + b * 2 + half) ^ swza) * 16) : koffa[b][1]));
        rb[b][0] = __builtin_bit_cast(u32x4, lds_read_b128(sb + koffb[b][0]));
        rb[b][1] = __builtin_bit_cast(u32x4, lds_read_b128(sb + koffb[b][1]));
    };
    auto wait_block = [&](int b) {
        asm volatile("s_waitcnt lgkmcnt(0)" ::: "memory");
        asm volatile("" : "+v"(ra[b][0]), "+v"(ra[b][1]), "+v"(rb[b][0]), "+v"(rb[b][1]));
    };
    auto products = [&](int b) {
        const f16x8 Ah = __builtin_bit_cast(f16x8, pln[0]), Al = __builtin_bit_cast(f16x8, pln[1]);
        acl = __builtin_amdgcn_mfma_f32_32x32x16_f16(Ah, __builtin_bit_cast(f16x8, rb[b][1]), acl, 0, 0, 0);
        acc = __builtin_amdgcn_mfma_f32_32x32x16_f16(Ah, __builtin_bit_cast(f16x8, rb[b][0]), acc, 0, 0, 0);
        acl = __builtin_amdgcn_mfma_f32_32x32x16_f16(Al, __builtin_bit_cast(f16x8, rb[b][0]), acl, 0, 0, 0);
    };
    const bool probe = p.dbg != nullptr && blockIdx.x == gridDim.x / 2 && wave_all == 0;
    unsigned long long treal0 = 0, tcyc0 = 0;
    if (probe) {
        treal0 = __builtin_amdgcn_s_memrealtime();
        tcyc0 = __builtin_readcyclecounter();
        if (lane == 0) p.dbg[9] = treal0 - t_entry;
    }
    int st = 0;
    for (int rd = 0; rd < nr; ++rd) {
        __builtin_amdgcn_s_barrier();
        asm volatile("" ::: "memory");
        const unsigned sa = a_lane + (unsigned)st * STAGE, sb = b_lane + (unsigned)st * STAGE;
        fetch(0, sa, sb);
        fetch(1, sa, sb);
        __builtin_amdgcn_sched_barrier(0);
        wait_block(0);
        wait_block(1);
        __builtin_amdgcn_sched_barrier(0);
        if constexpr (PRO == PRO_APL) { pln[0] = __builtin_bit_cast(u32x4, ra[0][0]); pln[1] = __builtin_bit_cast(u32x4, ra[0][1]); }
        else split2_f16<PRO>(ra[0][0], ra[0][1], pro_slope, pln[0], pln[1], amax);
        products(0);
        __builtin_amdgcn_sched_barrier(0);
        if constexpr (PRO == PRO_APL) { pln[0] = __builtin_bit_cast(u32x4, ra[1][0]); pln[1] = __builtin_bit_cast(u32x4, ra[1][1]); }
        else split2_f16<PRO>(ra[1][0], ra[1][1], pro_slope, pln[0], pln[1], amax);
        products(1);
        __builtin_amdgcn_sched_barrier(0);
        st = st + 1 == NST ? 0 : st + 1;
    }
    unsigned long long t_loop_end = 0;
    if (probe) {
        t_loop_end = __builtin_amdgcn_s_memrealtime();
        if (lane == 0) {
            p.dbg[6] = (unsigned long long)(nr * KS);
            p.dbg[7] = t_loop_end - treal0;
            p.dbg[8] = __builtin_readcyclecounter() - tcyc0;
        }
    }
    MT2_X3H_GUARD_RAISE(p, amax, lane);
#pragma unroll
    for (int e = 0; e < 16; ++e) acc[e] = __builtin_fmaf(acl[e], kX3hLoInv, acc[e]);
    if constexpr (KS > 1) {
        __syncthreads();
        float* red = smem + ((kg * NW + wave) * 16) * 64 + lane;
#pragma unroll
        for (int e = 0; e < 16; ++e) red[e * 64] = acc[e];
        __syncthreads();
        float out[EPG];
#pragma unroll
        for (int i = 0; i < EPG; ++i) {
            const int e = kg * EPG + i;
            float v = 0.0f;
#pragma unroll
            for (int g2 = 0; g2 < KS; ++g2) v += smem[(((g2 * NW + wave) * 16) + e) * 64 + lane];
            out[i] = v * inv_s;
        }
        if (lnx) {
            const int n = n0 + wn * 32 + (lane & 31);
            const float s_n = n < p.N ? p.ln_g[n] : 0.0f;
#pragma unroll
            for (int i = 0; i < EPG; ++i) {
                const int e = kg * EPG + i, rr = (e & 3) + 8 * (e >> 2) + 4 * half;
                out[i] = __shfl(ln_rs, rr) * (out[i] - __shfl(ln_mu, rr) * s_n);
            }
        }
        if (PRO == PRO_LNX && p.stat_out) epilogue_pre<EPG, PRO == PRO_LNX>(p, out, pre, g, m0 + wm * 32, n0 + wn * 32, lane, kg * EPG);
        else epilogue_pre<EPG>(p, out, pre, g, m0 + wm * 32, n0 + wn * 32, lane, kg * EPG);
    } else {
        float out[16];
#pragma unroll
        for (int e = 0; e < 16; ++e) out[e] = acc[e] * inv_s;
        if (lnx) {
            const int n = n0 + wn * 32 + (lane & 31);
            const float s_n = n < p.N ? p.ln_g[n] : 0.0f;
#pragma unroll
            for (int e = 0; e < 16; ++e) {
                const int rr = (e & 3) + 8 * (e >> 2) + 4 * half;
                out[e] = __shfl(ln_rs, rr) * (out[e] - __shfl(ln_mu, rr) * s_n);
            }
        }
        if (PRO == PRO_LNX && p.stat_out) epilogue_pre<16, PRO == PRO_LNX>(p, out, pre, g, m0 + wm * 32, n0 + wn * 32, lane, 0);
        else epilogue_pre<16>(p, out, pre, g, m0 + wm * 32, n0 + wn * 32, lane, 0);
    }
    if (probe) {
        __builtin_amdgcn_s_waitcnt(0);
        const unsigned long long t_end = __builtin_amdgcn_s_memrealtime();
        if (lane == 0) p.dbg[10] = t_end - t_loop_end;
    }
}

template <int QS, int BM, int BN, int WGM, int WGN, int NST, int PRO, int NL>
__global__ __launch_bounds__((WGM * WGN + NL) * 64) void conv_win_x3h_kernel(GemmP p) {
    using G = WinGeom<QS, BM, BN, WGM, WGN, NST, NL>;
    constexpr int NW = G::NW, WTM = G::WTM, WTN = G::WTN, TM = G::TM, TN = G::TN;
    constexpr int BPIECES = G::BPIECES, NI = NL, B_IT = G::B_IT, STAGE_B = G::STAGE_B;

    extern __shared__ __attribute__((aligned(16))) float smem[];
    const int tid = threadIdx.x, lane = tid & 63;
    const int wave_all = __builtin_amdgcn_readfirstlane(tid >> 6);
    const bool loader = wave_all >= NW;
    const int wave = loader ? wave_all - NW : wave_all;
    const int wm = wave / WGN, wn = wave % WGN;
    const int taps = p.taps, dil = p.dil;
    const int WR = BM + (taps - 1) * dil, WRp = (WR + 7) & ~7;
    char* ring = reinterpret_cast<char*>(smem);
    float* win = smem + NST * STAGE_B / 4;

    const int ntm = (p.M + BM - 1) / BM;
    const int tile = xcd_row_tile(blockIdx.x, ntm);
    const int m0 = tile * BM;

    const float* __restrict__ X = p.X;
    const char* __restrict__ Wh = reinterpret_cast<const char*>(p.Wh);
    const long long zoff_x = (const float*)g_zero16 - X;
    const long long zoff_w = (const char*)g_zero16 - Wh;
    const int ldx = p.ldx, Rx = p.Rx, Kt = p.K;

    {
        const int lrow = lane >> 3;
        const int ppq = WRp >> 3, pieces = QS * ppq;
        const int row_first = m0 + p.shift0;
        for (int pc = wave_all; pc < pieces; pc += NW + NL) {
            const int q = pc / ppq, r8 = pc - q * ppq;
            const int row = r8 * 8 + lrow;
            const int grow = row_first + row;
// ... 822 lines not shown
                fetch_b(b, sb);
                __builtin_amdgcn_sched_barrier(0);
            }
        }
        stn = stn + 1 == NST ? 0 : stn + 1;
        if (++qn == QS) { qn = 0; ++tapn; }
    };
    for (int c = 0; c + 1 < NK; ++c) chunk(std::false_type{});
    chunk(std::true_type{});
#pragma unroll
    for (int i = 0; i < TM; ++i)
#pragma unroll
        for (int j = 0; j < TN; ++j)
#pragma unroll
            for (int e = 0; e < 16; ++e) {
                float v = __builtin_fmaf(acl[i][j][e], kX3hLoInv, acc[i][j][e]) * inv_s[j];
                asm volatile("" : "+v"(v));
                acc[i][j][e] = v + bs[j];
            }
    GemmP e{};
    e.valid = p.valid; e.C = p.Y; e.ldc = p.ldy; e.M = p.R; e.N = BN; e.epi_act = ACT_NONE; e.out_scale = 1.0f;
    epilogue_t4<TM, TN>(e, acc, 0, m0 + wm * WTM, wn * WTN, lane);
}

typedef void (*UpMrfKernel)(UpMrfP);
struct UpMrfTile { int ch, bm, threads; size_t ring; UpMrfKernel fn; };
#define MT2_UPMRF_TILE(QS_, BM_, BN_, WM_, WN_, NST_, NL_)                                                                   \
    { BN_, BM_, WinGeom<QS_, BM_, BN_, WM_, WN_, NST_, NL_>::NT, WinGeom<QS_, BM_, BN_, WM_, WN_, NST_, NL_>::ring_bytes(),    \
      up_mrf_x3h_kernel<QS_, BM_, BN_, WM_, WN_, NST_, NL_> }
static const UpMrfTile kUpMrfTiles[2] = { MT2_UPMRF_TILE(2, 256, 64, 8, 1, 4, 4), MT2_UPMRF_TILE(4, 128, 128, 4, 2, 3, 4) };

UpMrfRoute up_mrf_route(const UpMrfP& p, const EngineOpts& o) {
    UpMrfRoute r{hipSuccess, -1, 0, 0, 0, 0};
    const auto fail = [&r](hipError_t e) { r.err = e; r.tile = -1; r.lds = 0; r.grid = r.block = 0; r.bm = 0; return r; };
    if (p.R <= 0) return r;
    const int t = p.ch == 64 ? 0 : (p.ch == 128 ? 1 : -1);
    if (t < 0 || p.stride != 2 || !((o.up_fuse >> t) & 1)) return fail(hipErrorNotSupported);
    if (!x3h_window_engine(o)) return fail(hipErrorNotSupported);
    if (!p.Wh || !p.inv) return fail(hipErrorNotSupported);
    if (!win_below_2g(p.R, p.ldx, p.ldy, p.ch, p.wh_ldb)) return fail(hipErrorNotSupported);
    if (!p.X0 || !p.X1 || !p.X2 || !p.Y || p.ldx < p.ch || p.ldy < p.ch || p.wh_ldb < 8ll * p.ch) return fail(hipErrorInvalidValue);
    if (!win_aligned(p.ldx, p.ldy, p.wh_ldb, (unsigned long long)p.Wh,
                     (unsigned long long)p.X0 | (unsigned long long)p.X1 | (unsigned long long)p.X2 | (unsigned long long)p.Y | (unsigned long long)p.bias))
        return fail(hipErrorNotSupported);
    const UpMrfTile& c = kUpMrfTiles[t];
    r.tile = t;
    r.bm = c.bm;
    r.lds = c.ring + win_lds_bytes(p.ch, c.bm, 2);
    r.grid = (unsigned)((p.R + c.bm - 1) / c.bm);
    r.block = (unsigned)c.threads;
    return r;
}

static std::atomic<unsigned long long> g_upmrf_attr_done[2];

hipError_t launch_up_mrf(const UpMrfP& p_in, hipStream_t s, EngineOpts* opts) {
    static const EngineOpts kDefaults;
    const EngineOpts& o = opts ? *opts : kDefaults;
    const UpMrfRoute r = up_mrf_route(p_in, o);
    if (r.err != hipSuccess || r.grid == 0) return r.err;
    const UpMrfTile& c = kUpMrfTiles[r.tile];
    UpMrfP p = p_in;
    p.x3h_flag = o.x3h_flag;
    p.ldr_prio = o.ldr_prio;
    const hipError_t e = dyn_lds_once(g_upmrf_attr_done[r.tile], reinterpret_cast<const void*>(c.fn), r.lds);
    if (e != hipSuccess) return e;
    if (opts) opts->last_cfg = "x3hupmrf";
    hipLaunchKernelGGL(c.fn, dim3(r.grid), dim3(r.block), r.lds, s, p);
    return hipGetLastError();
}


#define MT2_X3H_LDR(IDX_, BM_, BN_, WM_, WN_, NL_, NST_)                                                                    \
    { IDX_, BM_, BN_, (WM_* WN_ + NL_) * 64, (size_t)NST_ * ((size_t)BM_ * BK * 4 + (size_t)(2 * BN_ / 16) * 1024),         \
      "x3hldr" #BM_ "x" #BN_ "_" #WM_ "x" #WN_ "+" #NL_ "_s" #NST_ "xc",                                                    \
      { gemm_x3h_ldr_kernel<BM_, BN_, WM_, WN_, NL_, NST_, ACT_NONE>, gemm_x3h_ldr_kernel<BM_, BN_, WM_, WN_, NL_, NST_, ACT_RELU>, \
        gemm_x3h_ldr_kernel<BM_, BN_, WM_, WN_, NL_, NST_, ACT_LRELU>, gemm_x3h_ldr_kernel<BM_, BN_, WM_, WN_, NL_, NST_, PRO_APL>, \
        gemm_x3h_ldr_kernel<BM_, BN_, WM_, WN_, NL_, NST_, PRO_LNX> }, PIPE_X3H, 0, 0, (BN_) / (WN_) }
#define MT2_X3H_KS(IDX_, BM_, BN_, WM_, WN_, KS_, NL_, NST_)                                                                \
    { IDX_, BM_, BN_, (WM_* WN_ * KS_ + NL_) * 64, (size_t)KS_ * NST_ * ((size_t)BM_ * BK * 4 + (size_t)(2 * BN_ / 16) * 1024), \
      "x3hks" #BM_ "x" #BN_ "_" #WM_ "x" #WN_ "_k" #KS_ "+" #NL_ "_s" #NST_,                                                \
      { gemm_x3h_ks_kernel<BM_, BN_, WM_, WN_, KS_, NL_, NST_, ACT_NONE>, gemm_x3h_ks_kernel<BM_, BN_, WM_, WN_, KS_, NL_, NST_, ACT_RELU>, \
        gemm_x3h_ks_kernel<BM_, BN_, WM_, WN_, KS_, NL_, NST_, ACT_LRELU>, gemm_x3h_ks_kernel<BM_, BN_, WM_, WN_, KS_, NL_, NST_, PRO_APL>, \
        gemm_x3h_ks_kernel<BM_, BN_, WM_, WN_, KS_, NL_, NST_, PRO_LNX> }, PIPE_X3H, 0, KS_, 32 }
#define MT2_X3H_WIN(IDX_, QS_, BM_, BN_, WM_, WN_, NST_, NL_)                                                               \
    { IDX_, BM_, BN_, WinGeom<QS_, BM_, BN_, WM_, WN_, NST_, NL_>::NT, WinGeom<QS_, BM_, BN_, WM_, WN_, NST_, NL_>::ring_bytes(), \
      "x3hwin" #BM_ "x" #BN_ "_" #WM_ "x" #WN_ "+" #NL_ "_s" #NST_,                                                          \
      { conv_win_x3h_kernel<QS_, BM_, BN_, WM_, WN_, NST_, ACT_NONE, NL_>, conv_win_x3h_kernel<QS_, BM_, BN_, WM_, WN_, NST_, ACT_RELU, NL_>, \
        conv_win_x3h_kernel<QS_, BM_, BN_, WM_, WN_, NST_, ACT_LRELU, NL_> }, PIPE_X3H, QS_ }

static const TileCfg kX3hRows[] = {
    MT2_X3H_KS(CFG_X3HKS32x64_K4, 32, 64, 1, 2, 4, 8, 2),
    MT2_X3H_KS(CFG_X3HKS64x64_K2, 64, 64, 2, 2, 2, 8, 3),
    MT2_X3H_KS(CFG_X3HKS32x32_K8, 32, 32, 1, 1, 8, 8, 2),
    MT2_X3H_WIN(CFG_X3HWIN256x32, 1, 256, 32, 8, 1, 4, 4),
    MT2_X3H_WIN(CFG_X3HWIN256x64, 2, 256, 64, 8, 1, 4, 4),
    MT2_X3H_WIN(CFG_X3HWIN128x128, 4, 128, 128, 4, 2, 3, 4),
    MT2_X3H_LDR(CFG_X3HLDR128x128, 128, 128, 4, 2, 4, 4),
};
TileRows gemm_x3h_tile_rows() { return {kX3hRows, (int)(sizeof(kX3hRows) / sizeof(kX3hRows[0]))}; }

}
```

megatts2_amd/csrc/mt2_kernels.h:

```cpp
#pragma once
#include <hip/hip_runtime.h>
#include <stdint.h>

#include <atomic>
#include <vector>

namespace mt2 {

inline hipError_t dyn_lds_once(std::atomic<unsigned long long>& done, const void* fn, size_t bytes) {
    int dev = 0;
    hipError_t e = hipGetDevice(&dev);
    if (e != hipSuccess) return e;
    const unsigned long long bit = 1ull << (dev & 63);
    if (done.load(std::memory_order_acquire) & bit) return hipSuccess;
    e = hipFuncSetAttribute(fn, hipFuncAttributeMaxDynamicSharedMemorySize, (int)bytes);
    if (e != hipSuccess) return e;
    done.fetch_or(bit, std::memory_order_release);
    return hipSuccess;
}

constexpr int kInvalidRow = -(1 << 30);

enum Act : int { ACT_NONE = 0, ACT_RELU = 1, ACT_LRELU = 2, ACT_TANH = 3,
                 ACT_LOGCLAMP = 4 };

struct GemmP {
    const float* X; long long strideX; int ldx; int Rx;
    const int* rowbase; int a_mul; int shift0; int taps; int dil; int Cin;
    const float* W; long long strideW; int ldw;
    unsigned long long* dbg = nullptr;
    int epi_t4 = 1;
    int sk_nw = 8;
    int a_planes = 0;
    int c_planes = 0;
    int ldr64 = 0;
    int ldr_prio = 0;
    const void* W3 = nullptr;
    long long w3_plane = 0;
    const void* Wh = nullptr;
    long long wh_ldb = 0;
    long long wh_gstride = 0;
    const float* wh_inv = nullptr;
    long long wh_inv_stride = 0;
    int* x3h_flag = nullptr;
    const float* Wtm = nullptr;
    int tm_n0 = 0, tm_k0 = 0;
    int tm_kb = 0;
    const float* bias; long long strideB;
    const float* R; long long strideR; int ldr;
    const int* valid;
    float* C; long long strideC; int ldc;
    int M, N, K, groups;
    int pro_act; float pro_slope; int epi_act; float out_scale;
    const float* ln_g; const float* ln_b; float ln_eps;
    float* stat_out = nullptr; int stat_nt = 0, stat_w = 0;
    const float* ln_stat = nullptr; int ln_nt = 0, ln_w = 0;
};
struct TraceRec { int cfg; double flops; hipEvent_t e0, e1; int M, N, K, groups; };
struct EngineOpts {
    int force_cfg = -1;
    int t_ks4 = 256, t_ks2 = 640, t32 = 64, t32x32 = 160;
    bool splitk = true;
    int voc_streams = 3;
    bool win_conv = true;
    bool x6_conv = true;
    bool x6_gemm = true;
    int x3h = 15;
    int pair_fuse = 3;
    int up_fuse = 3;
    int* x3h_flag = nullptr;
    int t_x3h_128 = 72;
    int t_x6_256 = 160, t_x6_128 = 72;
    int x6_ks = 4;
    int a_planes = 3;
    bool ldr64 = false;
    int ldr_prio = 3;
    int skinny_rows = 64;
    int attn_lds_min = 640;
    int attn_x6_min = 192;
    bool skinny_tm = true;
    int skinny_pairs = 1;
    int skinny_nw = 16;
    bool markers = false;
    bool trace_on = false;
    std::vector<TraceRec> trace;
    const char* last_cfg = "";
    int last_stat_nt = 0, last_stat_w = 0;
    int last_sk_nw = 0;
    int ln_pairs = 0;
    int ln_pairs_adm = 2;
    int ln_pairs_maxk = 1024;
    int ln_pairs_maxm = 1280;
};
struct GemmRoute { hipError_t err; int cfg; int variant; size_t lds; int stat_nt, stat_w; };
GemmRoute gemm_route(const GemmP& p, const EngineOpts& o);
hipError_t launch_gemm(const GemmP& p, hipStream_t s, EngineOpts* o = nullptr);
struct PairP {
    const float* X; int ldx;
    int R, C, taps, dil;
    float slope;
    const void* Wh1; const float* inv1; const float* bias1;
    const void* Wh2; const float* inv2; const float* bias2;
    long long wh_ldb;
    const int* valid;
    float* Y; int ldy;
    int reflect = 0;
    int* x3h_flag = nullptr;
    int ldr_prio = 0;
};
struct PairRoute { hipError_t err; int tile; size_t lds; unsigned grid, block; int bm, bmo; };
PairRoute conv_pair_route(const PairP& p, const EngineOpts& o);
hipError_t launch_conv_pair(const PairP& p, hipStream_t s, EngineOpts* o = nullptr);
struct UpMrfP {
    const float* X0; const float* X1; const float* X2; int ldx;
    int R, ch, stride;
    float scale, slope;
    const void* Wh; const float* inv; const float* bias; long long wh_ldb;
    const int* valid;
    float* Y; int ldy;
    int* x3h_flag = nullptr;
    int ldr_prio = 0;
};
struct UpMrfRoute { hipError_t err; int tile; size_t lds; unsigned grid, block; int bm; };
UpMrfRoute up_mrf_route(const UpMrfP& p, const EngineOpts& o);
hipError_t launch_up_mrf(const UpMrfP& p, hipStream_t s, EngineOpts* o = nullptr);
bool gemm_takes_planes(const GemmP& p, const EngineOpts& o);
bool gemm_writes_planes(const GemmP& p, const EngineOpts& o);
bool gemm_skinny_eligible(const GemmP& p, int max_rows);
hipError_t launch_gemm_skinny(const GemmP& p, hipStream_t s);
bool gemm_skinny_tm_eligible(const GemmP& p, int max_rows);
hipError_t launch_gemm_skinny_tm(const GemmP& p, hipStream_t s);
int gemm_skinny_tm_waves(const GemmP& p);
hipError_t launch_tile_major(const float* W, int N, int K, float* out, hipStream_t s);
int gemm_num_configs();
const char* gemm_config_name(int idx);
int gemm_trace_collect(EngineOpts& o, int cap, const char** names, int64_t* launches, double* flops, double* ms);
int gemm_trace_shapes(EngineOpts& o, char* buf, int cap, int top);

struct LnP {
    const float* x; int ldx;
    const float* gamma; const float* beta; int rows_per_group;
    const float* R1; int ldr1; int r1_rows; const float* R2; int ldr2;
    const int* valid; int valid_rows;
    float* out; int ldo;
    int M, C; float eps; int act;
    int out_planes = 0;
    int* x3h_flag = nullptr;
};
hipError_t launch_layernorm(const LnP& p, hipStream_t s);

struct LnReduceP {
    const float* parts; long long pstride; int S;
    const float* bias; const float* R; int ldr;
    const float* gamma; const float* beta;
    float* xout; int ldx; float* hout; int ldh;
    int M, C; float eps;
    int h_planes = 0;
    int* x3h_flag = nullptr;
};
hipError_t launch_ln_reduce(const LnReduceP& p, hipStream_t s);

struct AttnP {
    const float* Q; int ldq; const float* K; int ldk; const float* V; int ldv;
    float* O; int ldo;
    const int* q_start; const int* q_len; const int* kv_start; const int* kv_len; const int* o_start;
    int u_qstride, u_qlen, u_kvstride, u_kvlen, u_ostride;
    int B, H, D, max_qlen; float scale;
    int max_kvlen;
    int lds_min_qlen = 640;
    int x6_min_qlen = 0;
    int lds_waves = 0;
    int ds_short = 1;
    int x3h = 0;
    int o_planes = 0;
    int* x3h_flag = nullptr;
};
enum AttnKernel {
// ... 271 lines not shown
```

megatts2_amd/runtime.py:

```python
from __future__ import annotations

import ctypes as C
import math
import os
from typing import Dict, Optional, Sequence

import numpy as np

from . import config as cfgmod
from . import sampling as sampmod

_LIB = None
MAX_POSITIONS = 8192

MT2_RUN_PLM, MT2_RUN_VOCODER, MT2_SKIP_ADM, MT2_PROMPT_VQPE = 1, 2, 4, 8
ACT_NONE, ACT_RELU, ACT_LRELU, ACT_TANH = 0, 1, 2, 3
ACT_LOGCLAMP = 4
MT2_RESAMPLE_NORMALIZE = 1
TRIM_FRAME, TRIM_HOP = 2048, 512
F0_FRAME, F0_WINDOW, F0_MAX_LAG = 1024, 768, 256
DTW_MAX_LEN, DTW_DIR_COLS = 4096, 16
PROSODY_FIELDS = 8
LOUDNESS_FIELDS = 8
EBU_FIELDS, TP_ZERO_CROSSINGS, TP_TAPS, TP_TILE = 18, 12, 24, 1024
# ... 1261 lines not shown


def op_layernorm_ex(x, ldx, gamma, beta, rows_per_group, R1, ldr1, r1_rows, R2, ldr2, valid, valid_rows, out, ldo, M, Cc, eps=1e-5,
                    act=ACT_NONE, out_planes=0, x3h_flag=None):
    _check(load_library().mt2_op_layernorm_ex(_stream(), _ptr(x), ldx, _ptr(gamma), _ptr(beta), rows_per_group, _ptr(R1), ldr1,
                                              r1_rows, _ptr(R2), ldr2, _ptr(valid), valid_rows, _ptr(out), ldo, M, Cc,
                                              C.c_float(eps), act, out_planes, _ptr(x3h_flag)))


def op_ln_reduce(parts, pstride, S, bias, R, ldr, gamma, beta, xout, ldx, hout, ldh, M, Cc, eps=1e-5, h_planes=0, x3h_flag=None):
    _check(load_library().mt2_op_ln_reduce(_stream(), _ptr(parts), C.c_longlong(pstride), S, _ptr(bias), _ptr(R), ldr, _ptr(gamma),
                                           _ptr(beta), _ptr(xout), ldx, _ptr(hout), ldh, M, Cc, C.c_float(eps), h_planes,
                                           _ptr(x3h_flag)))


def op_row(op, *args, stream=None):
    ptrs, ints, flts = [], [], []
    for a in args:
        if isinstance(a, float):
            flts.append(a)
        elif isinstance(a, (int, np.integer)) and not isinstance(a, bool):
            ints.append(int(a))
        else:
            ptrs.append(a.data_ptr() if a is not None else 0)
    _check(load_library().mt2_op_row(stream if stream is not None else _stream(), op.encode(), (C.c_void_p * len(ptrs))(*ptrs), len(ptrs),
                                     (C.c_longlong * len(ints))(*ints), len(ints), (C.c_float * len(flts))(*flts), len(flts)))


def op_embed_pe(table, Cc, ids, idmap, pos, pe, out, ldo, R, vocab): op_row("embed_pe", table, Cc, ids, idmap, pos, pe, out, ldo, R, vocab)
def op_gather_rows(src, lds_, map_, out, ldo, Cc, R): op_row("gather_rows", src, lds_, map_, out, ldo, Cc, R)
def op_pool_max(src, lds_, first, cnt, out, ldo, Cc, R): op_row("pool_max", src, lds_, first, cnt, out, ldo, Cc, R)
def op_sum_groups(x, strideG, groups, ld, out, ldo, Cc, R): op_row("sum_groups", x, strideG, groups, ld, out, ldo, Cc, R)
def op_avg3(a, b, d, scale, out, n): op_row("avg3", a, b, d, float(scale), out, n)
def op_conv_post(x0, x1, x2, scale, R, ch, k, w, bias, slope, valid, out): op_row("conv_post", x0, x1, x2, float(scale), R, ch, k, w, bias, float(slope), valid, out)
def op_fill_reflect(x, ld, Cc, start, len_, B, scale, G): op_row("fill_reflect", x, ld, Cc, start, len_, B, scale, G)
def op_pack_rows(src, Cc, Tmax, cmajor, rowmap, dst, ldd, R): op_row("pack_rows", src, Cc, Tmax, cmajor, rowmap, dst, ldd, R)
def op_unpack_rows(src, lds_, Cc, Tmax, cmajor, rowmap, dst, R): op_row("unpack_rows", src, lds_, Cc, Tmax, cmajor, rowmap, dst, R)
def op_adm_step_input(tc_emb, ld_tc, tc_row, w_dt, p, pstride, pe, x, Dc, De, n, A): op_row("adm_step_input", tc_emb, ld_tc, tc_row, w_dt, p, pstride, pe, x, Dc, De, n, A)
def op_plm_step_input(cond, ld_c, cond_row, emb, codes, cstride, pe, x, Dc, De, n, A, emb_rows): op_row("plm_step_input", cond, ld_c, cond_row, emb, codes, cstride, pe, x, Dc, De, n, A, emb_rows)
def op_adm_predict(x, D, w, p, pstride, n, xn, A): op_row("adm_predict", x, D, w, p, pstride, n, xn, A)
def op_adm_finalize(p, pstride, lens, slot_b, dur, flt, dstride, A, nmax): op_row("adm_finalize", p, pstride, lens, slot_b, dur, flt, dstride, A, nmax)
def op_plm_finalize(codes, cstride, lens, slot_b, out, ostride, A, nmax, skip): op_row("plm_finalize", codes, cstride, lens, slot_b, out, ostride, A, nmax, skip)
def op_adm_init_hist(p, pstride, prefix, P, slot_b, A): op_row("adm_init_hist", p, pstride, prefix, P, slot_b, A)
def op_plm_init_hist(codes, cstride, bos, prefix, P, pstride, slot_b, A): op_row("plm_init_hist", codes, cstride, bos, prefix, P, pstride, slot_b, A)
def op_check_ids(ids, map_, R, hi, flag, bit): op_row("check_ids", ids, map_, R, hi, flag, bit)
def op_copy_2d(src, spitch, dst, dpitch, width, rows): op_row("copy_2d", src, spitch, dst, dpitch, width, rows)
def op_scatter_i64(src, map_, out, R): op_row("scatter_i64", src, map_, out, R)
def op_expand_mask(in_, factor, out, n): op_row("expand_mask", in_, factor, out, n)
def op_unpack_wav(src, start, len_, out, out_stride, max_len, B): op_row("unpack_wav", src, start, len_, out, out_stride, max_len, B)
def op_argmax_rows(x, ldx, N, out, ostride, ooff, A): op_row("argmax_rows", x, ldx, N, out, ostride, ooff, A)
def op_vq_argmin(x, ldx, D, xe, ldxe, ee, N, valid, idx, M): op_row("vq_argmin", x, ldx, D, xe, ldxe, ee, N, valid, idx, M)
def op_row_sqnorm(E, D, ee, N): op_row("row_sqnorm", E, D, ee, N)
def op_codebook_rows(E, codes, codemap, out, ldo, Dq, R, bins): op_row("codebook_rows", E, codes, codemap, out, ldo, Dq, R, bins)
def op_reflect_pad_blocks(wav, wstride, blk_b, blk_t, len_, hop, pad, out, R): op_row("reflect_pad_blocks", wav, wstride, blk_b, blk_t, len_, hop, pad, out, R)
def op_magnitude(spec, lds_, F, out, ldo, M): op_row("magnitude", spec, lds_, F, out, ldo, M)
def op_gl_exp_rows(mel, Cc, rowmap, out, R): op_row("gl_exp_rows", mel, Cc, rowmap, out, R)
def op_gl_phase_init(A, lda, row_b, row_t, seeds, S, lds_, F, R): op_row("gl_phase_init", A, lda, row_b, row_t, seeds, S, lds_, F, R)
def op_istft_ola_blocks(frames, N, hop, w2, blk_b, blk_t, row0, T, out, Rb): op_row("istft_ola_blocks", frames, N, hop, w2, blk_b, blk_t, row0, T, out, Rb)
def op_istft_ola_wav(frames, N, hop, w2, row0, T, wav, L_max, B): op_row("istft_ola_wav", frames, N, hop, w2, row0, T, wav, L_max, B)
def op_gl_phase_update(R, Rprev, A, lda, S, lds_, F, c, resid, rmap, rows, update): op_row("gl_phase_update", R, Rprev, A, lda, S, lds_, F, float(c), resid, rmap, rows, update)



class MT2GemmDesc(C.Structure):
    _fields_ = [
        ("struct_bytes", C.c_int32),
        ("X", C.c_void_p), ("strideX", C.c_longlong), ("ldx", C.c_int32), ("Rx", C.c_int32),
        ("rowbase", C.c_void_p), ("a_mul", C.c_int32), ("shift0", C.c_int32), ("taps", C.c_int32), ("dil", C.c_int32),
        ("Cin", C.c_int32),
        ("W", C.c_void_p), ("strideW", C.c_longlong), ("ldw", C.c_int32),
        ("W3", C.c_void_p), ("w3_plane", C.c_longlong),
        ("Wh", C.c_void_p), ("wh_inv", C.c_void_p), ("wh_ldb", C.c_longlong), ("wh_gstride", C.c_longlong),
        ("wh_inv_stride", C.c_longlong),
        ("a_planes", C.c_int32),
        ("bias", C.c_void_p), ("strideB", C.c_longlong),
        ("R", C.c_void_p), ("strideR", C.c_longlong), ("ldr", C.c_int32),
        ("valid", C.c_void_p),
        ("C", C.c_void_p), ("strideC", C.c_longlong), ("ldc", C.c_int32),
        ("M", C.c_int32), ("N", C.c_int32), ("groups", C.c_int32),
        ("pro_act", C.c_int32), ("pro_slope", C.c_float), ("epi_act", C.c_int32), ("out_scale", C.c_float),
        ("force_cfg", C.c_int32),
        ("range_flag", C.c_void_p),
        ("cfg_out", C.POINTER(C.c_int32)),
    ]


def x3h_group_planes(row_len, w_off, ldw, strideW, groups):
    lib = load_library()
    form = C.c_int32(0)
    v = [C.c_longlong(0) for _ in range(5)]
    _check(lib.mt2_x3h_group_planes(C.c_longlong(row_len), C.c_longlong(w_off), C.c_longlong(ldw), C.c_longlong(strideW),
                                    C.c_longlong(groups), C.byref(form), *[C.byref(x) for x in v]))
    if form.value == 0:
        return None
    return {"form": {1: "whole", 2: "slices"}[form.value], "wh_off": v[0].value, "wh_ldb": v[1].value, "wh_gstride": v[2].value,
            "inv_off": v[3].value, "wh_inv_stride": v[4].value}


class GemmWeights:

    def __init__(self, W, device="cuda"):
        W = W.detach().to("cpu").contiguous()
        assert W.dim() == 2
        self.rows, self.row_len = W.shape
        self.f32 = W.to(device)
        self.w3 = split_bf16x3(W).to(device)
        ph, inv = split_f16x2_rows(W)
        self.ph, self.inv = ph.to(device), inv.to(device)


def op_gemm_grouped(X, wts, out, *, M, N, Cin, ldx, Rx, ldw, ldc, groups=1, strideX=0, strideW=0, strideC=0, w_off=0, taps=1, dil=1,
                    a_mul=1, shift0=0, rowbase=None, bias=None, strideB=0, R=None, strideR=0, ldr=0, valid=None, pro_act=ACT_NONE,
                    pro_slope=0.0, epi_act=ACT_NONE, out_scale=1.0, force_cfg=-1, x6=True, x3h=True, a_planes=0, wh_gstride=None,
                    flag=None):
    lib = load_library()
    d = MT2GemmDesc()
    d.struct_bytes = C.sizeof(MT2GemmDesc)
    d.X, d.strideX, d.ldx, d.Rx = X.data_ptr(), strideX, ldx, Rx
    d.rowbase = rowbase.data_ptr() if rowbase is not None else None
    d.a_mul, d.shift0, d.taps, d.dil, d.Cin = a_mul, shift0, taps, dil, Cin
    d.W, d.strideW, d.ldw = wts.f32.data_ptr() + 4 * w_off, strideW, ldw
    if x6:
        d.W3, d.w3_plane = wts.w3.data_ptr() + 2 * w_off, wts.rows * wts.row_len
    if x3h:
        g = x3h_group_planes(wts.row_len, w_off, ldw, strideW, groups)
        if g is not None:
            d.Wh, d.wh_inv = wts.ph.data_ptr() + g["wh_off"], wts.inv.data_ptr() + 4 * g["inv_off"]
            d.wh_ldb, d.wh_gstride, d.wh_inv_stride = g["wh_ldb"], g["wh_gstride"], g["wh_inv_stride"]
            if wh_gstride is not None:
                d.wh_gstride = wh_gstride
    d.a_planes = a_planes
    d.bias, d.strideB = (bias.data_ptr() if bias is not None else None), strideB
    d.R, d.strideR, d.ldr = (R.data_ptr() if R is not None else None), strideR, ldr
    d.valid = valid.data_ptr() if valid is not None else None
    d.C, d.strideC, d.ldc = out.data_ptr(), strideC, ldc
    d.M, d.N, d.groups = M, N, groups
    d.pro_act, d.pro_slope, d.epi_act, d.out_scale = pro_act, pro_slope, epi_act, out_scale
    d.force_cfg = force_cfg
    d.range_flag = flag.data_ptr() if flag is not None else None
    cfg = C.c_int32(-1)
    d.cfg_out = C.pointer(cfg)
    _check(lib.mt2_op_gemm_grouped(_stream(), C.byref(d)))
    return cfg.value


def op_attention(Q, K, V, q_start, q_len, kv_start, kv_len, H, D, scale, lds_min_qlen=-1, lds_waves=0, out=None, x6_min_qlen=-1):
    import torch
    lib = load_library()
    O = out if out is not None else torch.zeros(Q.shape[0], H * D, device=Q.device, dtype=torch.float32)
    B = q_start.shape[0]
    _check(lib.mt2_op_attention_tuned(_stream(), _ptr(Q), Q.stride(0), _ptr(K), K.stride(0), _ptr(V), V.stride(0), _ptr(O),
                                      O.stride(0), _ptr(q_start), _ptr(q_len), _ptr(kv_start), _ptr(kv_len), B, H, D,
                                      int(q_len.max().item()), C.c_float(scale), lds_min_qlen, lds_waves, x6_min_qlen,
                                      int(kv_len.max().item())))
    return O


def op_attention_x3h(Q, K, V, q_start, q_len, kv_start, kv_len, H, D, scale, lds_waves=0):
    import torch
    lib = load_library()
    O = torch.zeros(Q.shape[0], H * D, device=Q.device, dtype=torch.float32)
    flag = torch.zeros(4, device=Q.device, dtype=torch.int32)
    _check(lib.mt2_op_attention_x3h(_stream(), _ptr(Q), Q.stride(0), _ptr(K), K.stride(0), _ptr(V), V.stride(0), _ptr(O), O.stride(0),
                                    _ptr(q_start), _ptr(q_len), _ptr(kv_start), _ptr(kv_len), q_start.shape[0], H, D,
                                    int(q_len.max().item()), C.c_float(scale), lds_waves, int(kv_len.max().item()), _ptr(flag)))
    return O, int(flag[0].item())



ATTN_KERNELS = ("none", "generic", "reg", "ds", "lds", "x6", "x3h")


class MT2AttnDesc(C.Structure):
    _fields_ = [
        ("struct_bytes", C.c_int32),
        ("Q", C.c_void_p), ("ldq", C.c_int32),
        ("K", C.c_void_p), ("ldk", C.c_int32),
        ("V", C.c_void_p), ("ldv", C.c_int32),
        ("O", C.c_void_p), ("ldo", C.c_int32),
        ("q_start", C.c_void_p), ("q_len", C.c_void_p), ("kv_start", C.c_void_p), ("kv_len", C.c_void_p), ("o_start", C.c_void_p),
        ("u_qstride", C.c_int32), ("u_qlen", C.c_int32), ("u_kvstride", C.c_int32), ("u_kvlen", C.c_int32), ("u_ostride", C.c_int32),
        ("B", C.c_int32), ("H", C.c_int32), ("D", C.c_int32), ("max_qlen", C.c_int32), ("max_kvlen", C.c_int32), ("scale", C.c_float),
        ("lds_min_qlen", C.c_int32), ("x6_min_qlen", C.c_int32), ("lds_waves", C.c_int32), ("ds_short", C.c_int32),
        ("x3h", C.c_int32), ("o_planes", C.c_int32),
        ("range_flag", C.c_void_p),
        ("kernel_out", C.POINTER(C.c_int32)),
    ]


def _attn_desc(Q, ldq, K, ldk, V, ldv, O, ldo, *, B, H, D, max_qlen, scale, q_start=None, q_len=None, kv_start=None, kv_len=None,
               o_start=None, u_qstride=0, u_qlen=0, u_kvstride=0, u_kvlen=0, u_ostride=0, max_kvlen=0, lds_min_qlen, x6_min_qlen,
               lds_waves, ds_short, x3h, o_planes, flag=None):
    def addr(x):
        return None if x is None else (int(x) if isinstance(x, int) else x.data_ptr())
    d = MT2AttnDesc()
    d.struct_bytes = C.sizeof(MT2AttnDesc)
    d.Q, d.ldq, d.K, d.ldk, d.V, d.ldv, d.O, d.ldo = addr(Q), ldq, addr(K), ldk, addr(V), ldv, addr(O), ldo
    d.q_start, d.q_len, d.kv_start, d.kv_len, d.o_start = addr(q_start), addr(q_len), addr(kv_start), addr(kv_len), addr(o_start)
    d.u_qstride, d.u_qlen, d.u_kvstride, d.u_kvlen, d.u_ostride = u_qstride, u_qlen, u_kvstride, u_kvlen, u_ostride
    d.B, d.H, d.D, d.max_qlen, d.max_kvlen, d.scale = B, H, D, max_qlen, max_kvlen, scale
    d.lds_min_qlen, d.x6_min_qlen, d.lds_waves, d.ds_short, d.x3h, d.o_planes = lds_min_qlen, x6_min_qlen, lds_waves, ds_short, x3h, o_planes
    d.range_flag = addr(flag)
    return d


def op_attention_desc(Q, ldq, K, ldk, V, ldv, O, ldo, **geometry):
    d = _attn_desc(Q, ldq, K, ldk, V, ldv, O, ldo, **geometry)
    kernel = C.c_int32(0)
    d.kernel_out = C.pointer(kernel)
    _check(load_library().mt2_op_attention_desc(_stream(), C.byref(d)))
    return ATTN_KERNELS[kernel.value]


def attention_route(ldq, ldk, ldv, ldo, *, Q=128, K=128, V=128, O=128, **geometry):
    d = _attn_desc(Q, ldq, K, ldk, V, ldv, O, ldo, **geometry)
    err, kernel, lds = C.c_int32(0), C.c_int32(0), C.c_longlong(0)
    tmpl, launch = (C.c_int32 * 4)(), (C.c_int32 * 4)()
    if load_library().mt2_attention_route(C.byref(d), C.byref(err), C.byref(kernel), tmpl, launch, C.byref(lds)) != 0:
        raise NativeError("mt2_attention_route: null or mis-sized descriptor")
    return {"err": err.value, "kernel": ATTN_KERNELS[kernel.value], "d": tmpl[0], "nwq": tmpl[1], "nkv": tmpl[2], "nwv": tmpl[3],
            "grid": (launch[0], launch[1], launch[2]), "block": launch[3], "lds": lds.value}


def op_gemm_route(M, N, K, taps=1, dil=1, groups=1, pro_act=ACT_NONE, operands=0, misaligned=0, force_cfg=-1, x3h=15):
    out = [C.c_int(0), C.c_int(0), C.c_int(0), C.c_longlong(0), C.c_int(0)]
    _check(load_library().mt2_gemm_route(M, N, K, taps, dil, groups, pro_act, operands, misaligned, force_cfg, x3h, *map(C.byref, out)))
    return tuple(v.value for v in out)


def resample_query(sr_in: int, sr_out: int, L: int = 0):
    lo, o, n, k = C.c_longlong(0), C.c_int(0), C.c_int(0), C.c_int(0)
    _check(load_library().mt2_resample_query(int(sr_in), int(sr_out), int(L), C.byref(lo), C.byref(o), C.byref(n), C.byref(k)))
    return lo.value, o.value, n.value, k.value


def trim_query(L: int, top_db: float):
    f, c = C.c_int(0), C.c_float(0)
    _check(load_library().mt2_trim_query(int(L), float(top_db), C.byref(f), C.byref(c)))
    return f.value, np.float32(c.value)


def loudness_query(sample_rate: int, L: int):
    h, nb, ws = C.c_int(0), C.c_int(0), C.c_longlong(0)
    c = np.zeros(10, np.float64)
    _check(load_library().mt2_loudness_query(int(sample_rate), int(L), C.byref(h), C.byref(nb), c.ctypes.data_as(C.c_void_p), C.byref(ws)))
    return h.value, nb.value, c, ws.value


def ebu_query(sample_rate: int, L: int):
    o, taps, tile, nst, ws = C.c_int(0), C.c_int(0), C.c_int(0), C.c_int(0), C.c_longlong(0)
    _check(load_library().mt2_ebu_query(int(sample_rate), int(L), C.byref(o), C.byref(taps), C.byref(tile), C.byref(nst), C.byref(ws)))
    return o.value, taps.value, tile.value, nst.value, ws.value


def limiter_query(sample_rate: int, L: int, window_ms: float = 5.0):
    h, tile, ws = C.c_int(0), C.c_int(0), C.c_longlong(0)
    _check(load_library().mt2_limiter_query(int(sample_rate), int(L), float(window_ms), C.byref(h), C.byref(tile), C.byref(ws)))
    return h.value, tile.value, ws.value


def limiter_window(sample_rate: int, window_ms: float = 5.0):
    H = limiter_query(sample_rate, 1, window_ms)[0]
    w = np.zeros(2 * H + 1, np.float32)
    _check(load_library().mt2_limiter_window(int(sample_rate), float(window_ms), w.ctypes.data_as(C.c_void_p)))
    return w


def true_peak_table(sample_rate: int):
    o = ebu_query(sample_rate, 1)[0]
    table = np.zeros((o, TP_TAPS), np.float32)
    _check(load_library().mt2_true_peak_table(int(sample_rate), table.ctypes.data_as(C.c_void_p)))
    return table


def f0_query(L: int, sample_rate: int = 16000, hop: int = 256, fmin: float = 62.5, fmax: float = 500.0):
    f, lo, hi, ws = C.c_int(0), C.c_int(0), C.c_int(0), C.c_longlong(0)
    _check(load_library().mt2_f0_query(int(sample_rate), int(hop), float(fmin), float(fmax), int(L), C.byref(f), C.byref(lo), C.byref(hi),
                                       C.byref(ws)))
    return f.value, lo.value, hi.value, ws.value


def f0_track_query(L: int, B: int = 1, sample_rate: int = 16000, hop: int = 256, fmin: float = 62.5, fmax: float = 500.0,
                   octave_cost: float = 0.02, jump_cost: float = 0.5):
    f, lo, hi, n, ws = C.c_int(0), C.c_int(0), C.c_int(0), C.c_int(0), C.c_longlong(0)
    _check(load_library().mt2_f0_track_query(int(sample_rate), int(hop), float(fmin), float(fmax), float(octave_cost), float(jump_cost),
                                             int(L), int(B), C.byref(f), C.byref(lo), C.byref(hi), C.byref(n), C.byref(ws)))
    return f.value, lo.value, hi.value, n.value, ws.value


def dtw_query(Tx_max: int, Ty_max: int, D: int = 80, B: int = 1) -> int:
    n = C.c_longlong(0)
    _check(load_library().mt2_dtw_query(int(Tx_max), int(Ty_max), int(D), int(B), C.byref(n)))
    return n.value


def griffin_lim_query(audio, mel_lens=None, T_max: Optional[int] = None, B: Optional[int] = None, n_iter: int = 32,
                      momentum: float = 0.99, return_resid: bool = False):
    ac = MT2AudioConfig(audio.sample_rate, audio.n_fft, audio.hop_length, audio.win_length, audio.n_mels, audio.f_min, audio.f_max,
                        audio.clip)
    ln = None if mel_lens is None else _i32(mel_lens)
    if ln is not None:
        B = int(ln.size) if B is None else B
        T_max = int(ln.max()) if T_max is None and ln.size else T_max
    n, lo = C.c_longlong(0), C.c_longlong(0)
    _check(load_library().mt2_griffin_lim_query(C.byref(ac), _iptr(ln), int(T_max or 0), int(B or 0), int(n_iter), float(momentum),
                                                1 if return_resid else 0, C.byref(n), C.byref(lo)))
    return n.value, lo.value


def resample_table(sr_in: int, sr_out: int) -> np.ndarray:
    _, _, n, k = resample_query(sr_in, sr_out)
    h = np.empty((n, k), np.float32)
# ... 15 lines not shown
```

Baseline: 80500 mel-frames/s.

## Add row-major float4 epilogue for K-split x3h GEMM kernels

Adds an EPI4 variant of the K-split x3h GEMM kernel. The K-group partial sums are written to LDS as row-major images, reduced across K groups with float4 reads, and the result is stored through a vectorized epilogue that also handles bias, residual, valid mask and LN stats. The variant is selected at route time only when the N and leading dimensions are multiples of four and the pointers are 16-byte aligned. The goal is to replace scalar per-column stores and the shuffle-based reduction with coalesced 128-bit accesses, at the cost of twice as many kernel instantiations and a different summation order for the stats.

Measured after the change: 81530 mel-frames/s (median of 6 runs). 1.3% higher.

```diff
diff --git a/include/megatts2_hip.h b/include/megatts2_hip.h
--- a/include/megatts2_hip.h
+++ b/include/megatts2_hip.h
@@ -264,6 +264,8 @@
     int32_t force_cfg;
     int32_t* range_flag;
     int32_t* cfg_out;
+    int32_t ks_epi4;
+    int32_t* epi4_out;
 } mt2_gemm_desc;
 int mt2_op_gemm_grouped(void* stream, const mt2_gemm_desc* d);
 int mt2_x3h_guard(mt2_model* m, int* tripped);
@@ -329,6 +331,8 @@
 const char* mt2_gemm_config_name(int idx);
 int mt2_gemm_route(int M, int N, int K, int taps, int dil, int groups, int pro_act, int operands, int misaligned, int force_cfg,
                    int x3h, int* err, int* cfg, int* variant, long long* lds, int* planes);
+int mt2_gemm_route_ex(int M, int N, int K, int taps, int dil, int groups, int pro_act, int operands, int misaligned, int force_cfg,
+                      int x3h, int ld_pad, int ks_epi4, int* err, int* cfg, int* variant, long long* lds, int* planes, int* epi4);
 int mt2_conv_pair_route(int R, int C, int taps, int dil, int flags, int pair_fuse, int x3h, int* err, long long* lds, int* grid,
                         int* block, int* bm, int* bmo);
 int mt2_op_conv_pair(void* stream, const float* X, int ldx, int R, int C, int taps, int dil, float slope, const void* Wh1,
diff --git a/megatts2_amd/csrc/capi.inc b/megatts2_amd/csrc/capi.inc
--- a/megatts2_amd/csrc/capi.inc
+++ b/megatts2_amd/csrc/capi.inc
@@ -338,6 +338,7 @@
     if (n == "a_planes") return &m->opts.a_planes;
     if (n == "pair_fuse") return &m->opts.pair_fuse;
     if (n == "up_fuse") return &m->opts.up_fuse;
+    if (n == "ks_epi4") return &m->opts.ks_epi4;
     return nullptr;
 }
 static bool* option_flag(mt2_model* m, const std::string& n) {
@@ -1330,6 +1331,11 @@
 
 int mt2_gemm_route(int M, int N, int K, int taps, int dil, int groups, int pro_act, int operands, int misaligned, int force_cfg,
                    int x3h, int* err, int* cfg, int* variant, long long* lds, int* planes) {
+    return mt2_gemm_route_ex(M, N, K, taps, dil, groups, pro_act, operands, misaligned, force_cfg, x3h, 0, 1, err, cfg, variant, lds,
+                             planes, nullptr);
+}
+int mt2_gemm_route_ex(int M, int N, int K, int taps, int dil, int groups, int pro_act, int operands, int misaligned, int force_cfg,
+                      int x3h, int ld_pad, int ks_epi4, int* err, int* cfg, int* variant, long long* lds, int* planes, int* epi4) {
     alignas(128) static char dummy[12 * 128];
     const auto ptr = [&](int slot, int bit) { return (void*)(dummy + 128 * slot + ((misaligned & bit) ? 4 : 0)); };
     GemmP p{};
@@ -1347,10 +1353,15 @@
     if (operands & 64) p.rowbase = (const int*)ptr(11, 64);
     p.a_planes = (operands & 128) ? 1 : 0;
     p.c_planes = (operands & 256) ? 1 : 0;
+    p.ldc += ld_pad;
+    if (p.R) p.ldr += ld_pad;
+    p.strideC = (long long)M * p.ldc; p.strideR = (long long)M * p.ldc;
     EngineOpts o;
     o.force_cfg = force_cfg;
     o.x3h = x3h;
+    o.ks_epi4 = ks_epi4;
     const GemmRoute r = gemm_route(p, o);
+    if (epi4) *epi4 = r.ks_epi4;
     if (err) *err = (int)r.err;
     if (cfg) *cfg = r.cfg;
     if (variant) *variant = r.variant;
@@ -1483,6 +1494,7 @@
     p.ldc = ldc; p.M = M; p.N = N; p.K = taps * Cin; p.groups = 1; p.pro_act = pro_act; p.pro_slope = pro_slope; p.epi_act = epi_act;
     p.out_scale = 1.0f;
     EngineOpts o;
+    if (force_cfg >= 8000) { o.ks_epi4 = 0; force_cfg -= 8000; }
     if (force_cfg >= 4000) { p.c_planes = 1; force_cfg -= 4000; }
     if (force_cfg >= 2000) { p.a_planes = 1; force_cfg -= 2000; }
     o.ldr64 = force_cfg >= 1000;
@@ -1513,6 +1525,7 @@
     MT2_REQUIRE(d != nullptr, "null descriptor");
     MT2_REQUIRE(d->struct_bytes == (int32_t)sizeof(mt2_gemm_desc), "descriptor size mismatch");
     if (d->cfg_out) *d->cfg_out = -1;
+    if (d->epi4_out) *d->epi4_out = 0;
     GemmP p{};
     p.X = d->X; p.strideX = d->strideX; p.ldx = d->ldx; p.Rx = d->Rx;
     p.rowbase = d->rowbase; p.a_mul = d->a_mul; p.shift0 = d->shift0; p.taps = d->taps; p.dil = d->dil; p.Cin = d->Cin;
@@ -1528,7 +1541,10 @@
     EngineOpts o;
     o.force_cfg = d->force_cfg;
     o.x3h_flag = d->range_flag;
-    if (d->cfg_out) *d->cfg_out = gemm_route(p, o).cfg;
+    o.ks_epi4 = d->ks_epi4;
+    const GemmRoute rt = gemm_route(p, o);
+    if (d->cfg_out) *d->cfg_out = rt.cfg;
+    if (d->epi4_out) *d->epi4_out = rt.err == hipSuccess ? rt.ks_epi4 : 0;
     MT2_HIP(launch_gemm(p, (hipStream_t)stream, &o));
     MT2_API_END
 }
@@ -1563,6 +1579,7 @@
     p.epi_act = epi_act; p.out_scale = 1.0f; p.stat_out = stat_out;
     if (ln_stat) { p.pro_act = 5; p.ln_stat = ln_stat; p.ln_nt = ln_nt; p.ln_w = ln_w; p.ln_g = ln_s; p.ln_eps = ln_eps; }
     EngineOpts o;
+    if (force_cfg >= 8000) { o.ks_epi4 = 0; force_cfg -= 8000; }
     o.ldr64 = force_cfg >= 1000;
     o.force_cfg = force_cfg >= 1000 ? force_cfg - 1000 : force_cfg;
     const hipError_t e = launch_gemm(p, (hipStream_t)stream, &o);
@@ -1921,6 +1938,7 @@
     o.force_cfg = force_cfg;
     if (flags & 16) o.ldr_prio = 0;
     if (flags & 32) o.x3h = 0;
+    if (flags & 64) o.ks_epi4 = 0;
     hipError_t e = launch_gemm(p, s, &o);
     hipEvent_t e0, e1;
     MT2_HIP(hipEventCreate(&e0));
diff --git a/megatts2_amd/csrc/gemm_common.h b/megatts2_amd/csrc/gemm_common.h
--- a/megatts2_amd/csrc/gemm_common.h
+++ b/megatts2_amd/csrc/gemm_common.h
@@ -175,6 +175,88 @@
         if constexpr (STAT) { sv[i] = v; qv[i] = v * v; }
     }
     if constexpr (STAT) emit_row_pairs<NE>(p, sv, qv, mw, nw >> 5, 32.0f, lane, e0);
+}
+
+template <int NV> struct EpiPre4 { f32x4 r[NV]; int v[NV]; f32x4 b; };
+template <int NV>
+__device__ __forceinline__ void epi_prefetch4(const GemmP& p, EpiPre4<NV>& q, int g, int mw, int nw, int lane, int rl) {
+    const int n = nw + (lane & 7) * 4;
+    const bool nok = n < p.N;
+    const float* __restrict__ bias = p.bias ? p.bias + (long long)g * p.strideB + (nok ? n : 0) : g_zero16;
+    const float* __restrict__ R = p.R ? p.R + (long long)g * p.strideR + (nok ? n : 0) : g_zero16;
+    const long long ldr = p.R ? p.ldr : 0;
+    const int* __restrict__ vp = p.valid ? p.valid : g_one_i;
+    const int vs = p.valid ? 1 : 0;
+    q.b = *reinterpret_cast<const f32x4*>(bias);
+#pragma unroll
+    for (int v = 0; v < NV; ++v) {
+        int m = mw + rl + 8 * v;
+        m = m < p.M ? m : 0;
+        q.r[v] = *reinterpret_cast<const f32x4*>(R + m * ldr);
+        q.v[v] = vp[m * vs];
+    }
+}
+template <int NE>
+__device__ __forceinline__ float row4_sum32(float x0, float x1, float x2, float x3) {
+#pragma clang fp contract(off)
+    static_assert(NE == 2 || NE == 4 || NE == 8, "K-split shares of 2, 4 or 8 accumulator elements");
+    float s;
+    if constexpr (NE == 8) {
+        x0 += __shfl_xor(x0, 1); x1 += __shfl_xor(x1, 1); x2 += __shfl_xor(x2, 1); x3 += __shfl_xor(x3, 1);
+        s = (x0 + x2) + (x1 + x3);
+        s += __shfl_xor(s, 2);
+        s += __shfl_xor(s, 4);
+    } else {
+        if constexpr (NE == 4) s = (x0 + x2) + (x1 + x3);
+        else s = (x0 + x1) + (x2 + x3);
+        s += __shfl_xor(s, 1);
+        s += __shfl_xor(s, 2);
+        s += __shfl_xor(s, 4);
+    }
+    return s;
+}
+__device__ __forceinline__ float mul_uncontracted(float a, float b) {
+#pragma clang fp contract(off)
+    return a * b;
+}
+template <int NV, int NE, bool STAT = false>
+__device__ __forceinline__ void epilogue_pre4(const GemmP& p, const f32x4 (&acc)[NV], const EpiPre4<NV>& q, int g, int mw, int nw,
+                                              int lane, int rl, bool active) {
+    float* __restrict__ C = p.C + (long long)g * p.strideC;
+    const int epi_act = p.epi_act;
+    const float epi_par = p.pro_slope;
+    const float out_scale = p.out_scale;
+    const bool hasR = p.R != nullptr;
+    const int n = nw + (lane & 7) * 4;
+    const bool nok = n < p.N;
+#pragma unroll
+    for (int v = 0; v < NV; ++v) {
+        const int m = mw + rl + 8 * v;
+        f32x4 o = {0.f, 0.f, 0.f, 0.f};
+        if (active && nok && m < p.M) {
+#pragma unroll
+            for (int c = 0; c < 4; ++c) {
+                float x = acc[v][c] + q.b[c];
+                x = act_rt(epi_act, x, epi_par) * out_scale;
+                if (hasR) x += q.r[v][c];
+                if (q.v[v] == 0) x = 0.0f;
+                o[c] = x;
+            }
+            *reinterpret_cast<f32x4*>(C + (long long)m * p.ldc + n) = o;
+        }
+        if constexpr (STAT) {
+            const float S = row4_sum32<NE>(o[0], o[1], o[2], o[3]);
+            const float Q = row4_sum32<NE>(mul_uncontracted(o[0], o[0]), mul_uncontracted(o[1], o[1]), mul_uncontracted(o[2], o[2]),
+                                           mul_uncontracted(o[3], o[3]));
+            if (active && (lane & 7) == 0 && m < p.M) {
+                const float mean = S / 32.0f;
+                float2 pr;
+                pr.x = mean;
+                pr.y = fmaxf(Q - S * mean, 0.0f);
+                *reinterpret_cast<float2*>(p.stat_out + ((long long)m * p.stat_nt + (nw >> 5)) * 2) = pr;
+            }
+        }
+    }
 }
 
 template <int TM, int TN> struct EpiPreT { float r[TM][TN][16]; int v[TM][16]; float b[TN]; };
diff --git a/megatts2_amd/csrc/gemm_dispatch.hip b/megatts2_amd/csrc/gemm_dispatch.hip
--- a/megatts2_amd/csrc/gemm_dispatch.hip
+++ b/megatts2_amd/csrc/gemm_dispatch.hip
@@ -234,7 +234,7 @@
 
 GemmRoute gemm_route(const GemmP& p, const EngineOpts& o) {
     GemmRoute r{hipSuccess, -1, V_NONE, 0, 0, 0};
-    const auto fail = [&r](hipError_t e) { r.err = e; r.lds = 0; r.stat_nt = r.stat_w = 0; return r; };
+    const auto fail = [&r](hipError_t e) { r.err = e; r.lds = 0; r.stat_nt = r.stat_w = 0; r.ks_epi4 = 0; return r; };
     if (p.M <= 0 || p.N <= 0 || p.groups <= 0) return r;
     if ((p.Cin & 3) || (p.ldx & 3) || (p.ldw & 3) || p.K != p.taps * p.Cin) return fail(hipErrorInvalidValue);
     if (p.pro_act < 0 || p.pro_act > PRO_LNX) return fail(hipErrorInvalidValue);
@@ -297,6 +297,12 @@
         r.lds = c->lds + (size_t)c->win_qs * wrp * BK * sizeof(float);
     }
     if (!c->fn[r.variant]) return fail(hipErrorNotSupported);
+    if (o.ks_epi4 && x3h && c->x6_ks && c->fn4[r.variant]) {
+        const auto on16 = [](const void* q) { return (((unsigned long long)q) & 15) == 0; };
+        const bool grp4 = p.groups == 1 || ((p.strideC | (p.R ? p.strideR : 0) | (p.bias ? p.strideB : 0) | p.wh_inv_stride) & 3) == 0;
+        r.ks_epi4 = ((p.N | p.ldc | (p.R ? p.ldr : 0)) & 3) == 0 && grp4 && on16(p.C) && on16(p.R) && on16(p.bias) && on16(p.wh_inv) &&
+                    (p.pro_act != PRO_LNX || on16(p.ln_g));
+    }
     return r;
 }
 
@@ -320,14 +326,14 @@
     return c_planes_ok(p, *cfg_table().row[choose_cfg(p, o)], p.stat_out != nullptr);
 }
 
-static std::atomic<unsigned long long> g_attr_done[kNumCfgs][kGemmVariants];
+static std::atomic<unsigned long long> g_attr_done[kNumCfgs][2 * kGemmVariants];
 
 hipError_t launch_gemm(const GemmP& p_in, hipStream_t s, EngineOpts* opts) {
     static const EngineOpts kDefaults;
     const EngineOpts& o = opts ? *opts : kDefaults;
     const GemmRoute r = gemm_route(p_in, o);
     if (r.cfg < 0 && r.err == hipSuccess) return hipSuccess;
-    if (opts) { opts->last_stat_nt = r.stat_nt; opts->last_stat_w = r.stat_w; opts->last_sk_nw = 0; }
+    if (opts) { opts->last_stat_nt = r.stat_nt; opts->last_stat_w = r.stat_w; opts->last_sk_nw = 0; opts->last_ks_epi4 = r.ks_epi4; }
     if (r.err != hipSuccess) return r.err;
     GemmP p = p_in;
     if (!r.stat_nt) p.stat_out = nullptr;
@@ -345,9 +351,9 @@
         p.x3h_flag = o.x3h_flag;
     }
     if (c->pipe == PIPE_X6 && p.w3_plane == 0) p.w3_plane = (long long)p.N * p.ldw;
-    const GemmKernel fn = c->fn[r.variant];
+    const GemmKernel fn = r.ks_epi4 ? c->fn4[r.variant] : c->fn[r.variant];
     const size_t lds_attr = c->win_qs ? c->lds + (size_t)c->win_qs * ((c->bm + 64 + 7) & ~7) * BK * sizeof(float) : r.lds;
-    const hipError_t e = dyn_lds_once(g_attr_done[r.cfg][r.variant], reinterpret_cast<const void*>(fn), lds_attr);
+    const hipError_t e = dyn_lds_once(g_attr_done[r.cfg][r.variant + (r.ks_epi4 ? kGemmVariants : 0)], reinterpret_cast<const void*>(fn), lds_attr);
     if (e != hipSuccess) return e;
     const int tiles = ((p.M + c->bm - 1) / c->bm) * ((p.N + c->bn - 1) / c->bn);
     p.epi_t4 = 1;
diff --git a/megatts2_amd/csrc/gemm_tiles.h b/megatts2_amd/csrc/gemm_tiles.h
--- a/megatts2_amd/csrc/gemm_tiles.h
+++ b/megatts2_amd/csrc/gemm_tiles.h
@@ -45,6 +45,7 @@
     int win_qs = 0;
     int x6_ks = 0;
     int stat_w = 0;
+    GemmKernel fn4[kGemmVariants] = {};
 };
 struct TileRows { const TileCfg* rows; int n; };
 TileRows gemm_f32_tile_rows();
diff --git a/megatts2_amd/csrc/gemm_x3h.hip b/megatts2_amd/csrc/gemm_x3h.hip
--- a/megatts2_amd/csrc/gemm_x3h.hip
+++ b/megatts2_amd/csrc/gemm_x3h.hip
@@ -533,7 +533,7 @@
     }
 }
 
-template <int BM, int BN, int WGM, int WGN, int KS, int NL, int NST, int PRO>
+template <int BM, int BN, int WGM, int WGN, int KS, int NL, int NST, int PRO, bool EPI4 = false>
 __global__ __launch_bounds__((WGM * WGN * KS + NL) * 64) void gemm_x3h_ks_kernel(GemmP p) {
     constexpr int NW = WGM * WGN;
     constexpr int NWC = NW * KS;
@@ -542,6 +542,8 @@
     constexpr int LW = PT / NL;
     constexpr int STAGE_A = BM * BK * 4, STAGE_B = PB * 1024, STAGE = STAGE_A + STAGE_B;
     constexpr int EPG = 16 / KS;
+    constexpr int NV = EPG >= 4 ? EPG / 4 : 1;
+    static_assert(!EPI4 || KS > 1, "the row-major finish reads the K-group reduction's LDS images");
     static_assert(BM == 32 * WGM && BN == 32 * WGN, "one 32x32 tile per wave");
     static_assert(PT % NL == 0 && 16 % KS == 0 && NST >= 2 && (NST - 2) * LW < 64 && NWC + NL <= 16, "config");
     static_assert(KS * NST * STAGE >= NWC * 16 * 64 * 4 || KS == 1, "the K-group reduction reuses the ring");
@@ -648,15 +650,24 @@
 
     const int kg = wave_all / NW, wave = wave_all % NW;
     const int wm = wave / WGN, wn = wave % WGN;
-    EpiPre<EPG> pre;
-    epi_prefetch<EPG>(p, pre, g, m0 + wm * 32, n0 + wn * 32, lane, kg * EPG);
+    EpiPre<EPI4 ? 1 : EPG> pre;
+    EpiPre4<NV> pre4;
     float inv_s;
-    {
+    f32x4 inv4, sn4;
+    const bool lnx = PRO == PRO_LNX && p.pro_act == PRO_LNX;
+    const bool active4 = EPG >= 4 || lane < 32;
+    const int rl4 = active4 ? kg * 2 * EPG + (lane >> 3) : 0;
+    if constexpr (EPI4) {
+        epi_prefetch4<NV>(p, pre4, g, m0 + wm * 32, n0 + wn * 32, lane, rl4);
+        const int n = n0 + wn * 32 + (lane & 7) * 4;
+        inv4 = *reinterpret_cast<const f32x4*>(p.wh_inv + (long long)g * p.wh_inv_stride + (n < p.N ? n : 0));
+        sn4 = *reinterpret_cast<const f32x4*>(lnx ? p.ln_g + (n < p.N ? n : 0) : g_zero16);
+    } else {
+        epi_prefetch<EPG>(p, pre, g, m0 + wm * 32, n0 + wn * 32, lane, kg * EPG);
         const int n = n0 + wn * 32 + (lane & 31);
         inv_s = (p.wh_inv + (long long)g * p.wh_inv_stride)[n < p.N ? n : 0];
     }
     float ln_mu = 0.0f, ln_rs = 0.0f;
-    const bool lnx = PRO == PRO_LNX && p.pro_act == PRO_LNX;
     if (lnx) lnx_row_stats<2>(p, m0 + wm * 32 + (lane & 31), lane >> 5, 32, ln_mu, ln_rs);
     f32x16 acc, acl;
 #pragma unroll
@@ -736,7 +747,36 @@
     MT2_X3H_GUARD_RAISE(p, amax, lane);
 #pragma unroll
     for (int e = 0; e < 16; ++e) acc[e] = __builtin_fmaf(acl[e], kX3hLoInv, acc[e]);
-    if constexpr (KS > 1) {
+    if constexpr (EPI4) {
+        __syncthreads();
+        float* img = smem + (kg * NW + wave) * 1024 + half * 128 + (lane & 31);
+#pragma unroll
+        for (int e = 0; e < 16; ++e) img[((e & 3) + 8 * (e >> 2)) * 32] = acc[e];
+        __syncthreads();
+        f32x4 out[NV];
+#pragma unroll
+        for (int v = 0; v < NV; ++v) {
+            f32x4 s = {0.f, 0.f, 0.f, 0.f};
+#pragma unroll
+            for (int g2 = 0; g2 < KS; ++g2) {
+                const f32x4 t = *reinterpret_cast<const f32x4*>(smem + (g2 * NW + wave) * 1024 + (rl4 + 8 * v) * 32 + (lane & 7) * 4);
+#pragma unroll
+                for (int c = 0; c < 4; ++c) s[c] += t[c];
+            }
+#pragma unroll
+            for (int c = 0; c < 4; ++c) out[v][c] = s[c] * inv4[c];
+        }
+        if (lnx) {
+#pragma unroll
+            for (int v = 0; v < NV; ++v) {
+                const float rs = __shfl(ln_rs, rl4 + 8 * v), mu = __shfl(ln_mu, rl4 + 8 * v);
+#pragma unroll
+                for (int c = 0; c < 4; ++c) out[v][c] = rs * (out[v][c] - mu * sn4[c]);
+            }
+        }
+        if (PRO == PRO_LNX && p.stat_out) epilogue_pre4<NV, EPG, PRO == PRO_LNX>(p, out, pre4, g, m0 + wm * 32, n0 + wn * 32, lane, rl4, active4);
+        else epilogue_pre4<NV, EPG>(p, out, pre4, g, m0 + wm * 32, n0 + wn * 32, lane, rl4, active4);
+    } else if constexpr (KS > 1) {
         __syncthreads();
         float* red = smem + ((kg * NW + wave) * 16) * 64 + lane;
 #pragma unroll
@@ -1725,7 +1765,10 @@
       "x3hks" #BM_ "x" #BN_ "_" #WM_ "x" #WN_ "_k" #KS_ "+" #NL_ "_s" #NST_,                                                \
       { gemm_x3h_ks_kernel<BM_, BN_, WM_, WN_, KS_, NL_, NST_, ACT_NONE>, gemm_x3h_ks_kernel<BM_, BN_, WM_, WN_, KS_, NL_, NST_, ACT_RELU>, \
         gemm_x3h_ks_kernel<BM_, BN_, WM_, WN_, KS_, NL_, NST_, ACT_LRELU>, gemm_x3h_ks_kernel<BM_, BN_, WM_, WN_, KS_, NL_, NST_, PRO_APL>, \
-        gemm_x3h_ks_kernel<BM_, BN_, WM_, WN_, KS_, NL_, NST_, PRO_LNX> }, PIPE_X3H, 0, KS_, 32 }
+        gemm_x3h_ks_kernel<BM_, BN_, WM_, WN_, KS_, NL_, NST_, PRO_LNX> }, PIPE_X3H, 0, KS_, 32,                            \
+      { gemm_x3h_ks_kernel<BM_, BN_, WM_, WN_, KS_, NL_, NST_, ACT_NONE, true>, gemm_x3h_ks_kernel<BM_, BN_, WM_, WN_, KS_, NL_, NST_, ACT_RELU, true>, \
+        gemm_x3h_ks_kernel<BM_, BN_, WM_, WN_, KS_, NL_, NST_, ACT_LRELU, true>, gemm_x3h_ks_kernel<BM_, BN_, WM_, WN_, KS_, NL_, NST_, PRO_APL, true>, \
+        gemm_x3h_ks_kernel<BM_, BN_, WM_, WN_, KS_, NL_, NST_, PRO_LNX, true> } }
 #define MT2_X3H_WIN(IDX_, QS_, BM_, BN_, WM_, WN_, NST_, NL_)                                                               \
     { IDX_, BM_, BN_, WinGeom<QS_, BM_, BN_, WM_, WN_, NST_, NL_>::NT, WinGeom<QS_, BM_, BN_, WM_, WN_, NST_, NL_>::ring_bytes(), \
       "x3hwin" #BM_ "x" #BN_ "_" #WM_ "x" #WN_ "+" #NL_ "_s" #NST_,                                                          \
diff --git a/megatts2_amd/csrc/mt2_kernels.h b/megatts2_amd/csrc/mt2_kernels.h
--- a/megatts2_amd/csrc/mt2_kernels.h
+++ b/megatts2_amd/csrc/mt2_kernels.h
@@ -73,6 +73,7 @@
     int t_x6_256 = 160, t_x6_128 = 72;
     int x6_ks = 4;
     int a_planes = 3;
+    int ks_epi4 = 1;
     bool ldr64 = false;
     int ldr_prio = 3;
     int skinny_rows = 64;
@@ -86,13 +87,14 @@
     std::vector<TraceRec> trace;
     const char* last_cfg = "";
     int last_stat_nt = 0, last_stat_w = 0;
+    int last_ks_epi4 = 0;
     int last_sk_nw = 0;
     int ln_pairs = 0;
     int ln_pairs_adm = 2;
     int ln_pairs_maxk = 1024;
     int ln_pairs_maxm = 1280;
 };
-struct GemmRoute { hipError_t err; int cfg; int variant; size_t lds; int stat_nt, stat_w; };
+struct GemmRoute { hipError_t err; int cfg; int variant; size_t lds; int stat_nt, stat_w; int ks_epi4; };
 GemmRoute gemm_route(const GemmP& p, const EngineOpts& o);
 hipError_t launch_gemm(const GemmP& p, hipStream_t s, EngineOpts* o = nullptr);
 struct PairP {
diff --git a/megatts2_amd/runtime.py b/megatts2_amd/runtime.py
--- a/megatts2_amd/runtime.py
+++ b/megatts2_amd/runtime.py
@@ -1367,6 +1367,8 @@
         ("force_cfg", C.c_int32),
         ("range_flag", C.c_void_p),
         ("cfg_out", C.POINTER(C.c_int32)),
+        ("ks_epi4", C.c_int32),
+        ("epi4_out", C.POINTER(C.c_int32)),
     ]
 
 
@@ -1397,7 +1399,7 @@
 def op_gemm_grouped(X, wts, out, *, M, N, Cin, ldx, Rx, ldw, ldc, groups=1, strideX=0, strideW=0, strideC=0, w_off=0, taps=1, dil=1,
                     a_mul=1, shift0=0, rowbase=None, bias=None, strideB=0, R=None, strideR=0, ldr=0, valid=None, pro_act=ACT_NONE,
                     pro_slope=0.0, epi_act=ACT_NONE, out_scale=1.0, force_cfg=-1, x6=True, x3h=True, a_planes=0, wh_gstride=None,
-                    flag=None):
+                    flag=None, ks_epi4=1, want_epi4=False):
     lib = load_library()
     d = MT2GemmDesc()
     d.struct_bytes = C.sizeof(MT2GemmDesc)
@@ -1423,10 +1425,11 @@
     d.pro_act, d.pro_slope, d.epi_act, d.out_scale = pro_act, pro_slope, epi_act, out_scale
     d.force_cfg = force_cfg
     d.range_flag = flag.data_ptr() if flag is not None else None
-    cfg = C.c_int32(-1)
+    cfg, epi4 = C.c_int32(-1), C.c_int32(0)
     d.cfg_out = C.pointer(cfg)
+    d.ks_epi4, d.epi4_out = ks_epi4, C.pointer(epi4)
     _check(lib.mt2_op_gemm_grouped(_stream(), C.byref(d)))
-    return cfg.value
+    return (cfg.value, epi4.value) if want_epi4 else cfg.value
 
 
 def op_attention(Q, K, V, q_start, q_len, kv_start, kv_len, H, D, scale, lds_min_qlen=-1, lds_waves=0, out=None, x6_min_qlen=-1):
@@ -1513,6 +1516,13 @@
     return tuple(v.value for v in out)
 
 
+def op_gemm_route_ex(M, N, K, taps=1, dil=1, groups=1, pro_act=ACT_NONE, operands=0, misaligned=0, force_cfg=-1, x3h=15, ld_pad=0, ks_epi4=1):
+    out = [C.c_int(0), C.c_int(0), C.c_int(0), C.c_longlong(0), C.c_int(0), C.c_int(0)]
+    _check(load_library().mt2_gemm_route_ex(M, N, K, taps, dil, groups, pro_act, operands, misaligned, force_cfg, x3h, ld_pad, ks_epi4,
+                                            *map(C.byref, out)))
+    return tuple(v.value for v in out)
+
+
 def resample_query(sr_in: int, sr_out: int, L: int = 0):
     lo, o, n, k = C.c_longlong(0), C.c_int(0), C.c_int(0), C.c_int(0)
     _check(load_library().mt2_resample_query(int(sr_in), int(sr_out), int(L), C.byref(lo), C.byref(o), C.byref(n), C.byref(k)))
```
